# seung-lab/crackle

Hardware: AMD Instinct MI355X
Metric: voxels/s encode+decode, 1024x1024x512 uint32; bit-exact .ckl bytes (higher is better)
Workload: dtype u32

## Files before the change

crackle_amd/_lib.py:

```python
import ctypes as C
import os

HERE = os.path.dirname(os.path.abspath(__file__))
LIB_PATH = os.path.join(HERE, "libcrackle_amd_tuning.so" if os.environ.get("CKL_TUNING_LIB") else
                        ("libcrackle_amd_%s.so" % os.environ["CKL_LIB_AB"]) if os.environ.get("CKL_LIB_AB") else "libcrackle_amd.so")

CKL_OK, CKL_ERR_FORMAT, CKL_ERR_RUNTIME, CKL_ERR_ARG, CKL_ERR_NO_DEVICE, CKL_ERR_CRC = range(6)
MEM_HOST, MEM_DEVICE = 0, 1
CKL_DUST_BINARY_IMAGE, CKL_DUST_INVERT = 1, 2
CKL_ERODE_KEEP_BORDER = 1


class HeaderInfo(C.Structure):
  _fields_ = [
    ("format_version", C.c_uint32), ("label_format", C.c_uint32), ("crack_format", C.c_uint32),
    ("is_signed", C.c_uint32), ("data_width", C.c_uint32), ("stored_data_width", C.c_uint32),
    ("sx", C.c_uint32), ("sy", C.c_uint32), ("sz", C.c_uint32),
    ("fortran_order", C.c_uint32), ("markov_model_order", C.c_uint32), ("is_sorted", C.c_uint32),
    ("num_label_bytes", C.c_uint64), ("header_bytes", C.c_uint64),
  ]


MERGE_UNIQUE_FN = C.CFUNCTYPE(C.c_int, C.c_void_p, C.POINTER(C.c_uint64), C.c_uint64, C.POINTER(C.c_void_p), C.POINTER(C.c_uint64))


class EncodeOverrides(C.Structure):
  _fields_ = [
    ("force_crack_format", C.c_int32), ("force_label_format", C.c_int32),
    ("force_stored_width", C.c_int32), ("has_model", C.c_int32),
    ("model", C.c_void_p),
    ("merge_unique", MERGE_UNIQUE_FN), ("merge_ctx", C.c_void_p),
  ]


EXPORTS = {
  "ckl_last_error": (C.c_char_p, []),
  "ckl_abi_version": (C.c_int, []),
  "ckl_device_count": (C.c_int, []),
  "ckl_header_info_from_bytes": (C.c_int, [C.c_char_p, C.c_uint64, C.POINTER(HeaderInfo)]),
  "ckl_compress": (C.c_int, [
    C.c_void_p, C.c_int, C.c_int, C.c_int, C.c_int64, C.c_int64, C.c_int64,
    C.c_int, C.c_int, C.c_uint64, C.c_int, C.c_int, C.c_int64,
    C.c_int, C.POINTER(C.c_void_p), C.POINTER(C.c_uint64)]),
  "ckl_free": (None, [C.c_void_p]),
  "ckl_decompress": (C.c_int, [
    C.c_void_p, C.c_uint64, C.c_void_p, C.c_uint64, C.c_int,
    C.c_int64, C.c_int64, C.c_int, C.c_uint64, C.c_int]),
  "ckl_decoder_create": (C.c_int, [C.c_void_p, C.c_uint64, C.c_int64, C.c_int64, C.c_int, C.POINTER(C.c_void_p)]),
  "ckl_decoder_create_device": (C.c_int, [C.c_void_p, C.c_uint64, C.c_int64, C.c_int64, C.c_int, C.POINTER(C.c_void_p)]),
  "ckl_encoder_keep_device_stream": (C.c_int, [C.c_void_p, C.c_int]),
  "ckl_encoder_async_host_copy": (C.c_int, [C.c_void_p, C.c_int]),
  "ckl_encoder_host_wait": (C.c_int, [C.c_void_p]),
  "ckl_encoder_device_stream": (C.c_int, [C.c_void_p, C.POINTER(C.c_void_p), C.POINTER(C.c_uint64)]),
  "ckl_decoder_run": (C.c_int, [C.c_void_p, C.c_void_p, C.c_uint64, C.c_int, C.c_uint64]),
  "ckl_decoder_cutout": (C.c_int, [C.c_void_p, C.c_int64, C.c_int64, C.c_int64, C.c_int64, C.c_void_p, C.c_uint64, C.c_int, C.c_uint64]),
  "ckl_cutout": (C.c_int, [
    C.c_void_p, C.c_uint64, C.c_void_p, C.c_uint64, C.c_int,
    C.c_int64, C.c_int64, C.c_int64, C.c_int64, C.c_int64, C.c_int64, C.c_int, C.c_uint64, C.c_int]),
  "ckl_paste": (C.c_int, [
    C.c_void_p, C.c_uint64, C.c_void_p, C.c_int, C.c_int, C.c_uint64,
    C.c_int64, C.c_int64, C.c_int64, C.c_int64, C.c_int64, C.c_int64,
    C.c_int, C.POINTER(C.c_void_p), C.POINTER(C.c_uint64)]),
  "ckl_decoder_label_stats": (C.c_int, [C.c_void_p, C.c_uint64, C.c_void_p, C.c_void_p, C.c_void_p, C.c_void_p, C.POINTER(C.c_uint64)]),
  "ckl_decoder_contacts": (C.c_int, [C.c_void_p, C.POINTER(C.c_void_p), C.POINTER(C.c_void_p), C.POINTER(C.c_uint64)]),
  "ckl_decoder_overlaps": (C.c_int, [C.c_void_p, C.c_void_p, C.POINTER(C.c_void_p), C.POINTER(C.c_void_p), C.POINTER(C.c_uint64)]),
  "ckl_overlaps": (C.c_int, [
    C.c_void_p, C.c_uint64, C.c_void_p, C.c_uint64, C.c_int64, C.c_int64, C.c_int,
    C.POINTER(C.c_void_p), C.POINTER(C.c_void_p), C.POINTER(C.c_uint64)]),
  "ckl_decoder_last_timing": (C.c_int, [C.c_void_p, C.POINTER(C.c_float), C.POINTER(C.c_float)]),
  "ckl_decoder_stage_timing": (C.c_int, [C.c_void_p, C.c_int, C.POINTER(C.c_char_p), C.POINTER(C.c_float)]),
  "ckl_decoder_set_stage_events": (C.c_int, [C.c_void_p, C.c_int]),
  "ckl_decoder_destroy": (None, [C.c_void_p]),
  "ckl_encoder_create": (C.c_int, [C.c_int64, C.c_int64, C.c_int64, C.c_int, C.c_int, C.POINTER(C.c_void_p)]),
  "ckl_encoder_run": (C.c_int, [
    C.c_void_p, C.c_void_p, C.c_int64, C.c_int64, C.c_int64,
    C.c_int, C.c_int, C.c_uint64, C.c_int, C.c_int, C.c_int64,
    C.POINTER(EncodeOverrides), C.POINTER(C.c_void_p), C.POINTER(C.c_uint64)]),
  "ckl_encoder_stats": (C.c_int, [
    C.c_void_p, C.c_void_p, C.c_int64, C.c_int64, C.c_int64,
    C.POINTER(C.c_uint64), C.POINTER(C.c_uint64), C.POINTER(C.c_uint64), C.POINTER(C.c_uint64)]),
  "ckl_encoder_markov_stats": (C.c_int, [
    C.c_void_p, C.c_void_p, C.c_int64, C.c_int64, C.c_int64, C.c_int, C.c_uint64, C.c_void_p]),
  "ckl_encoder_components": (C.c_int, [
    C.c_void_p, C.c_void_p, C.c_int64, C.c_int64, C.c_int64, C.c_uint32, C.c_void_p, C.c_void_p]),
  "ckl_encoder_components_device": (C.c_int, [
    C.c_void_p, C.c_void_p, C.c_int64, C.c_int64, C.c_int64, C.c_uint32, C.c_void_p, C.c_void_p]),
  "ckl_encoder_pin_labels": (C.c_int, [
    C.c_void_p, C.c_void_p, C.c_void_p, C.c_int64, C.c_int64, C.c_int64, C.c_void_p,
    C.c_int, C.c_int, C.c_int64, C.POINTER(C.c_void_p), C.POINTER(C.c_uint64)]),
  "ckl_pins_rows_first": (C.c_int, [C.c_void_p, C.c_void_p, C.c_void_p, C.c_int64, C.c_int64, C.c_int64, C.c_int64, C.c_uint64, C.c_void_p, C.c_void_p, C.c_void_p]),
  "ckl_pins_rows_best": (C.c_int, [C.c_void_p, C.c_void_p, C.c_void_p, C.c_int64, C.c_int64, C.c_int64, C.c_int64, C.c_uint64, C.c_void_p, C.c_void_p]),
  "ckl_pins_rows_extent": (C.c_int, [C.c_void_p, C.c_void_p, C.c_void_p, C.c_int64, C.c_int64, C.c_int64, C.c_int64, C.c_uint64, C.c_void_p, C.c_void_p, C.c_void_p, C.c_void_p]),
  "ckl_pins_rows_ids": (C.c_int, [C.c_void_p, C.c_void_p, C.c_int64, C.c_int64, C.c_int64, C.c_int64, C.c_uint64, C.c_void_p, C.c_void_p, C.c_void_p, C.c_void_p]),
  "ckl_pins_rows_section": (C.c_int, [C.c_void_p, C.c_int64, C.c_int64, C.c_int64, C.c_uint64, C.c_void_p, C.c_void_p, C.c_void_p, C.c_void_p, C.c_void_p, C.c_void_p, C.c_void_p,
                                       C.c_int, C.c_int, C.c_int64, C.POINTER(C.c_void_p), C.POINTER(C.c_uint64)]),
  "ckl_encoder_walk_step_kinds": (C.c_int, [C.c_void_p, C.POINTER(C.c_uint32), C.c_uint32, C.POINTER(C.c_uint32)]),
  "ckl_encoder_last_timing": (C.c_int, [C.c_void_p, C.POINTER(C.c_float), C.POINTER(C.c_float)]),
  "ckl_encoder_walk_paths": (C.c_int, [C.c_void_p, C.POINTER(C.c_uint32), C.POINTER(C.c_uint32)]),
  "ckl_encoder_emit_path": (C.c_int, [C.c_void_p, C.POINTER(C.c_int), C.POINTER(C.c_uint64)]),
  "ckl_encoder_destroy": (None, [C.c_void_p]),
  "ckl_pin_labels_host": (C.c_int, [
    C.c_void_p, C.c_int, C.c_void_p, C.c_int64, C.c_int64, C.c_int64, C.c_void_p,
    C.c_int, C.c_int, C.c_int64, C.POINTER(C.c_void_p), C.POINTER(C.c_uint64)]),
  "ckl_zstack": (C.c_int, [C.POINTER(C.c_char_p), C.POINTER(C.c_uint64), C.c_uint64, C.POINTER(C.c_void_p), C.POINTER(C.c_uint64)]),
  "ckl_decoder_check": (C.c_int, [C.c_void_p, C.c_void_p, C.c_uint64]),
  "ckl_decoder_vcg": (C.c_int, [C.c_void_p, C.c_void_p, C.c_uint64, C.c_int]),
  "ckl_voxel_connectivity_graph": (C.c_int, [C.c_void_p, C.c_uint64, C.c_int, C.c_int, C.c_void_p, C.c_uint64]),
  "ckl_voxel_connectivity_graph_range": (C.c_int, [C.c_void_p, C.c_uint64, C.c_int64, C.c_int64, C.c_int, C.c_int, C.c_void_p, C.c_uint64]),
  "ckl_point_cloud": (C.c_int, [
    C.c_void_p, C.c_uint64, C.c_int64, C.c_int64, C.c_void_p, C.c_uint64, C.c_int, C.c_int, C.c_int,
    C.POINTER(C.c_void_p), C.POINTER(C.c_void_p), C.POINTER(C.c_void_p), C.POINTER(C.c_uint64)]),
  "ckl_reencode_markov": (C.c_int, [C.c_void_p, C.c_uint64, C.c_int, C.c_int, C.POINTER(C.c_void_p), C.POINTER(C.c_uint64)]),
  "ckl_recompress": (C.c_int, [C.c_void_p, C.c_uint64, C.c_int, C.c_int, C.POINTER(C.c_void_p), C.POINTER(C.c_uint64)]),
  "ckl_erode": (C.c_int, [C.c_void_p, C.c_uint64, C.c_int, C.c_int, C.c_int, C.c_int, C.POINTER(C.c_void_p), C.POINTER(C.c_uint64)]),
  "ckl_dilate": (C.c_int, [C.c_void_p, C.c_uint64, C.c_int, C.c_int, C.c_int, C.c_int, C.POINTER(C.c_void_p), C.POINTER(C.c_uint64)]),
  "ckl_decoder_crack_planes": (C.c_int, [C.c_void_p, C.POINTER(C.c_void_p), C.POINTER(C.c_void_p), C.POINTER(C.c_uint32), C.POINTER(C.c_uint64)]),
  "ckl_zsplit": (C.c_int, [C.c_void_p, C.c_uint64, C.c_int64, C.c_int64, C.POINTER(C.c_void_p), C.POINTER(C.c_uint64)]),
  "ckl_encoder_defer_codes": (C.c_int, [C.c_void_p, C.c_int]),
  "ckl_encoder_codes_to_host": (C.c_int, [C.c_void_p, C.c_void_p, C.c_uint64, C.POINTER(C.c_uint64)]),
  "ckl_host_register": (C.c_int, [C.c_void_p, C.c_uint64]),
  "ckl_host_unregister": (C.c_int, [C.c_void_p]),
  "ckl_array_equal": (C.c_int, [C.c_void_p, C.c_uint64, C.c_void_p, C.c_uint64, C.c_int, C.POINTER(C.c_int)]),
  "ckl_mode_pooling_2x2x1": (C.c_int, [C.c_void_p, C.c_uint64, C.c_int64, C.c_int64, C.c_int, C.POINTER(C.c_void_p), C.POINTER(C.c_uint64), C.POINTER(C.c_void_p), C.POINTER(C.c_uint64)]),
  "ckl_connected_components": (C.c_int, [C.c_void_p, C.c_uint64, C.c_int, C.c_int, C.POINTER(C.c_void_p), C.POINTER(C.c_uint64), C.POINTER(C.c_void_p), C.POINTER(C.c_uint64)]),
  "ckl_relabel_components": (C.c_int, [C.c_void_p, C.c_uint64, C.c_void_p, C.c_uint64, C.POINTER(C.c_void_p), C.POINTER(C.c_uint64)]),
  "ckl_dust": (C.c_int, [C.c_void_p, C.c_uint64, C.c_uint64, C.c_int, C.c_int, C.c_int, C.POINTER(C.c_void_p), C.POINTER(C.c_uint64), C.POINTER(C.c_uint64)]),
  "ckl_fill_holes": (C.c_int, [C.c_void_p, C.c_uint64, C.c_int, C.c_int, C.POINTER(C.c_void_p), C.POINTER(C.c_uint64), C.POINTER(C.c_uint64)]),
  "ckl_relabel_values": (C.c_int, [C.c_void_p, C.c_uint64, C.c_void_p, C.c_uint64, C.POINTER(C.c_void_p), C.POINTER(C.c_uint64)]),
  "ckl_crc32c": (C.c_uint32, [C.c_void_p, C.c_uint64]),
  "ckl_crc32c_combine": (C.c_uint32, [C.c_uint32, C.c_uint32, C.c_uint64]),
}

_lib = None


def lib():
  global _lib
  if _lib is None:
    if not os.path.exists(LIB_PATH):
      raise ImportError(
        f"{LIB_PATH} is missing: build the HIP extension first "
        "(python -m crackle_amd.build, or __graft_entry__.build()). "
        "crackle_amd has no CPU fallback."
      )
    L = C.CDLL(LIB_PATH)
    for name, (res, args) in EXPORTS.items():
      f = getattr(L, name)
      f.restype = res
      f.argtypes = args
    _lib = L
  return _lib


def last_error() -> str:
  return lib().ckl_last_error().decode("utf-8", "replace")


class HostStream:

  def __init__(self, ptr: int, n: int):
    self.ptr, self.n = int(ptr), int(n)

  def __len__(self):
    return self.n

  def view(self) -> memoryview:
    return memoryview((C.c_ubyte * self.n).from_address(self.ptr)).cast("B")

  def tobytes(self) -> bytes:
    return C.string_at(self.ptr, self.n)

  __bytes__ = tobytes

  def __eq__(self, other):
    if isinstance(other, HostStream):
      return self.tobytes() == other.tobytes()
    if isinstance(other, (bytes, bytearray, memoryview)):
      return self.tobytes() == bytes(other)
    return NotImplemented

  def __del__(self):
    try:
# ... 12 lines not shown
```

crackle_amd/csrc/ckl_encode.hip:

```cpp
#include "ckl_encoder.hpp"
#include "ckl_decoder.hpp"
#include "ckl_runs.hpp"
#include "ckl_strips.hpp"
#include "ckl_trail.hpp"
#include "ckl_code_words.hpp"
#include "ckl_recompress.hpp"

#include <algorithm>
#include <atomic>
#include <chrono>
#include <functional>
#include <memory>
#include <mutex>

namespace ckl {

using namespace dev;

template <typename LABEL>
__global__ void __launch_bounds__(kBlock) k_stats(const LABEL* __restrict__ labels, uint64_t voxels, unsigned long long* __restrict__ out ) {
	__shared__ unsigned long long s_max[kWaves], s_pairs[kWaves];
	unsigned long long mx = 0, pairs = 0;
	const uint64_t stride = static_cast<uint64_t>(gridDim.x) * kBlock;
	for (uint64_t i = static_cast<uint64_t>(blockIdx.x) * kBlock + threadIdx.x; i < voxels; i += stride) {
// ... 32 lines not shown
	const uint32_t unit0 = (blockIdx.x * kWaves + wave) * kPlaneUnroll;
	const LABEL* slice = labels + static_cast<uint64_t>(zi) * sy * sx;
	LABEL v[kPlaneUnroll], up[kPlaneUnroll], lf[kPlaneUnroll];
	uint32_t xs[kPlaneUnroll], ys[kPlaneUnroll];
#pragma unroll
	for (uint32_t k = 0; k < kPlaneUnroll; k++) {
		const uint32_t unit = unit0 + k;
		const uint32_t y = unit / chunks_per_row;
		const uint32_t x = (unit - y * chunks_per_row) * 64u + lane;
		xs[k] = x; ys[k] = y;
		const bool valid = unit < units && x < sx;
		const LABEL* row = slice + static_cast<uint64_t>(y) * sx;
		v[k] = valid ? row[x] : LABEL(0);
		up[k] = (valid && y > 0) ? row[static_cast<int64_t>(x) - static_cast<int64_t>(sx)] : v[k];
		lf[k] = (valid && lane == 0 && x > 0) ? row[x - 1] : v[k];
	}
	uint32_t nv = 0, nh = 0;
#pragma unroll
	for (uint32_t k = 0; k < kPlaneUnroll; k++) {
		const uint32_t unit = unit0 + k;
		const bool valid = unit < units && xs[k] < sx;
		LABEL left = __shfl_up(v[k], 1, kWave);
		if (lane == 0) left = lf[k];
		const bool dv = valid && xs[k] > 0 && v[k] != left;
		const bool dh = valid && v[k] != up[k];
		const unsigned long long mv = __ballot(dv), mh = __ballot(dh);
		if (lane == 0 && unit < units) {
			const uint32_t c = xs[k] >> 6;
			const uint64_t wbase = zi * plane_words + static_cast<uint64_t>(ys[k]) * row_words + c * 2u;
			planeV[wbase] = static_cast<uint32_t>(mv);
			planeH[wbase] = static_cast<uint32_t>(mh);
			if (c * 2u + 1u < row_words) {
				planeV[wbase + 1] = static_cast<uint32_t>(mv >> 32);
				planeH[wbase + 1] = static_cast<uint32_t>(mh >> 32);
			}
			nv += __popcll(mv);
			nh += __popcll(mh);
		}
	}
	if (lane == 0) { s_red[wave] = nv; s_red[kWaves + wave] = nh; }
	__syncthreads();
	if (threadIdx.x == 0) {
		uint32_t tv = 0, th = 0;
		for (int w = 0; w < kWaves; w++) { tv += s_red[w]; th += s_red[kWaves + w]; }
		if (tv) atomicAdd(count_v + zi, tv);
		if (th) atomicAdd(count_h + zi, th);
	}
}

constexpr uint32_t kBandRows = 32;

template <typename V, typename T>
__device__ __forceinline__ V nt_load_vec(const T* p) {
	typedef uint32_t u32x4_t __attribute__((ext_vector_type(4)));
	static_assert(sizeof(V) == 16, "one 16-byte vector");
	const u32x4_t raw = __builtin_nontemporal_load(reinterpret_cast<const u32x4_t*>(p));
	V v;
	__builtin_memcpy(&v, &raw, 16);
	return v;
}

template <typename T>
__device__ __forceinline__ T wave_shift_up1_label(T v) {
	if constexpr (sizeof(T) == 8) {
		const uint32_t lo = dev::wave_shift_up1(static_cast<uint32_t>(v), 0u), hi = dev::wave_shift_up1(static_cast<uint32_t>(static_cast<uint64_t>(v) >> 32), 0u);
		return static_cast<T>((static_cast<uint64_t>(hi) << 32) | lo);
	}
	else return static_cast<T>(dev::wave_shift_up1(static_cast<uint32_t>(v), 0u));
}
template <uint32_t G>
__device__ __forceinline__ uint32_t or_over_lane_group(uint32_t v) {
	static_assert(G == 2 || G == 4 || G == 8 || G == 16, "lane groups inside a row of 16");
	if constexpr (G >= 2) v |= dev::dpp_u32<0xB1, 0xF>(0u, v);
	if constexpr (G >= 4) v |= dev::dpp_u32<0x4E, 0xF>(0u, v);
	if constexpr (G >= 8) v |= dev::dpp_u32<0x141, 0xF>(0u, v);
	if constexpr (G >= 16) v |= dev::dpp_u32<0x140, 0xF>(0u, v);
	return v;
}

template <typename LABEL>
__global__ void __launch_bounds__(kBlock) k_label_planes_stream(
	const LABEL* __restrict__ labels, uint32_t sx, uint32_t sy, uint32_t strips, uint32_t bands,
	uint32_t* __restrict__ planeV, uint32_t* __restrict__ planeH, uint32_t row_words, uint64_t plane_words,
	uint32_t* __restrict__ partial, unsigned long long* __restrict__ partial_max, unsigned long long* __restrict__ total_pairs
) {
	if (blockIdx.x == 0 && blockIdx.y == 0 && threadIdx.x == 0) *total_pairs = 0;
	constexpr uint32_t P = 16 / sizeof(LABEL);
	constexpr uint32_t G = 32 / P;
	constexpr uint32_t WPR = 64 / G;
	struct alignas(16) Vec { LABEL v[P]; };
	__shared__ uint32_t s_red[3 * kWaves];
	__shared__ unsigned long long s_max[kWaves];
	__shared__ __attribute__((aligned(16))) uint32_t s_words[kWaves][2][kBandRows * WPR];
	const uint32_t zi = blockIdx.y;
	const uint32_t lane = threadIdx.x & 63u, wave = threadIdx.x >> 6;
	const uint32_t task = blockIdx.x * kWaves + wave;
	uint32_t nv = 0, nh = 0, pairs = 0;
	LABEL mxl = 0;
	if (task < strips * bands) {
		const uint32_t band = __builtin_amdgcn_readfirstlane(task / strips), strip = __builtin_amdgcn_readfirstlane(task - (task / strips) * strips);
		const uint32_t x0 = strip * (64u * P);
		const uint32_t x = x0 + lane * P;
		const uint32_t y0 = band * kBandRows, y1 = min(y0 + kBandRows, sy);
		const bool active = x < sx;
		const uint64_t slice_off = static_cast<uint64_t>(zi) * sy * sx;
		const LABEL* col = labels + slice_off + (active ? x : 0u);
		Vec prev;
#pragma unroll
		for (uint32_t i = 0; i < P; i++) prev.v[i] = 0;
		if (y0 > 0) prev = nt_load_vec<Vec>(col + static_cast<uint64_t>(y0 - 1) * sx);
		uint32_t* sv = s_words[wave][0];
		uint32_t* sh = s_words[wave][1];
		auto edge_of = [&](uint32_t y, bool& have) -> LABEL {
			const uint64_t lin = slice_off + static_cast<uint64_t>(y) * sx + x0;
			have = lin > 0;
			const uint64_t at = have ? lin - 1 : 0;
			if constexpr (sizeof(LABEL) >= 4) return labels[at];
			else {
				const uint64_t byte = at * sizeof(LABEL);
				const uint32_t w = reinterpret_cast<const uint32_t*>(reinterpret_cast<uintptr_t>(labels) & ~static_cast<uintptr_t>(3))[(byte + (reinterpret_cast<uintptr_t>(labels) & 3u)) >> 2];
				return static_cast<LABEL>(w >> (8u * static_cast<uint32_t>((byte + (reinterpret_cast<uintptr_t>(labels) & 3u)) & 3u)));
			}
		};
		constexpr uint32_t kRowsAhead = 4;
		Vec rows[kRowsAhead];
		LABEL edges[kRowsAhead];
		bool have_edges[kRowsAhead];
		auto request = [&](uint32_t r, uint32_t y) {
			const uint32_t yl = y < y1 ? y : y1 - 1u;
			rows[r] = nt_load_vec<Vec>(col + static_cast<uint64_t>(yl) * sx);
			edges[r] = edge_of(yl, have_edges[r]);
		};
#pragma unroll
		for (uint32_t r = 0; r < kRowsAhead; r++) request(r, y0 + r);
#pragma unroll
		for (uint32_t it = 0; it < kBandRows / kRowsAhead; it++) {
			const uint32_t yb = y0 + it * kRowsAhead;
#pragma unroll
			for (uint32_t r = 0; r < kRowsAhead; r++) {
				const uint32_t y = yb + r;
				const Vec cur = rows[r];
				const LABEL edge = edges[r];
				const bool have_edge = have_edges[r];
				request(r, y + kRowsAhead);
				if (y >= y1) continue;
				LABEL left = wave_shift_up1_label(cur.v[P - 1]);
				bool have_left = true;
				if (lane == 0) { left = edge; have_left = have_edge; }
				uint32_t bv = 0, bh = 0;
				if (active) {
#pragma unroll
					for (uint32_t i = 0; i < P; i++) {
						const LABEL l = i ? cur.v[i - 1] : left;
						bv |= (cur.v[i] != l ? 1u : 0u) << i;
						bh |= (cur.v[i] != prev.v[i] ? 1u : 0u) << i;
						mxl = cur.v[i] > mxl ? cur.v[i] : mxl;
					}
					pairs += P - __popc(bv) - ((have_left || (bv & 1u)) ? 0u : 1u);
					if (x == 0) bv &= ~1u;
					if (y == 0) bh = 0u;
				}
				nv += __popc(bv); nh += __popc(bh);
				bv <<= (lane % G) * P; bh <<= (lane % G) * P;
				bv = or_over_lane_group<G>(bv); bh = or_over_lane_group<G>(bh);
				if ((lane % G) == 0) { sv[(y - y0) * WPR + lane / G] = bv; sh[(y - y0) * WPR + lane / G] = bh; }
				prev = cur;
			}
		}
		const uint32_t word0 = x0 >> 5;
		uint32_t* pv = planeV + zi * plane_words;
		uint32_t* ph = planeH + zi * plane_words;
		constexpr uint32_t kVecWords = WPR >= 4 ? 4u : WPR;
		constexpr uint32_t kLanesPerRow = WPR / kVecWords;
		for (uint32_t r0 = 0; r0 < y1 - y0; r0 += 64u / kLanesPerRow) {
			const uint32_t r = r0 + lane / kLanesPerRow, w = (lane % kLanesPerRow) * kVecWords;
			if (r >= y1 - y0) continue;
			const uint64_t at = static_cast<uint64_t>(y0 + r) * row_words + word0 + w;
			if (word0 + w + kVecWords <= row_words && ((at & (kVecWords - 1u)) == 0u) && kVecWords == 4u) {
				*reinterpret_cast<uint4*>(pv + at) = *reinterpret_cast<const uint4*>(sv + r * WPR + w);
				*reinterpret_cast<uint4*>(ph + at) = *reinterpret_cast<const uint4*>(sh + r * WPR + w);
			}
			else {
				for (uint32_t q = 0; q < kVecWords; q++) if (word0 + w + q < row_words) { pv[at + q] = sv[r * WPR + w + q]; ph[at + q] = sh[r * WPR + w + q]; }
			}
		}
	}
	nv = wave_sum(nv); nh = wave_sum(nh); pairs = wave_sum(pairs);
	unsigned long long mx = static_cast<unsigned long long>(mxl);
	for (int d = kWave / 2; d >= 1; d >>= 1) { const unsigned long long o = __shfl_xor(mx, d, kWave); mx = o > mx ? o : mx; }
	if (lane == 0) { s_red[wave] = nv; s_red[kWaves + wave] = nh; s_red[2 * kWaves + wave] = pairs; s_max[wave] = mx; }
	__syncthreads();
	if (threadIdx.x == 0) {
		uint32_t tv = 0, th = 0, tp = 0;
		unsigned long long tm = 0;
		for (int w = 0; w < kWaves; w++) { tv += s_red[w]; th += s_red[kWaves + w]; tp += s_red[2 * kWaves + w]; tm = s_max[w] > tm ? s_max[w] : tm; }
		const uint64_t o = static_cast<uint64_t>(zi) * gridDim.x + blockIdx.x;
		partial[o * 4 + 0] = tv; partial[o * 4 + 1] = th; partial[o * 4 + 2] = tp; partial[o * 4 + 3] = 0;
		partial_max[o] = tm;
	}
}

__global__ void __launch_bounds__(kBlock) k_planes_from_cracks(
	const uint32_t* __restrict__ crackV, const uint32_t* __restrict__ crackH, uint32_t sx, uint32_t sy,
	uint32_t row_words, uint64_t plane_words, uint32_t permissible,
	uint32_t* __restrict__ planeV, uint32_t* __restrict__ planeH, uint32_t* __restrict__ counts, uint32_t nslices
) {
	__shared__ uint32_t s_red[kWaves];
	const uint32_t zi = blockIdx.y;
	const uint64_t i = static_cast<uint64_t>(blockIdx.x) * kBlock + threadIdx.x;
	uint32_t nv = 0, nh = 0;
	if (i < plane_words) {
		const uint32_t y = static_cast<uint32_t>(i / row_words);
		const uint32_t w = static_cast<uint32_t>(i - static_cast<uint64_t>(y) * row_words);
		const uint32_t left = sx - w * 32u;
		const uint32_t in_row = left >= 32u ? 0xFFFFFFFFu : ((1u << left) - 1u);
		const uint32_t mv = in_row & (w == 0 ? 0xFFFFFFFEu : 0xFFFFFFFFu);
		const uint32_t mh = y >= 1 ? in_row : 0u;
		const uint64_t at = zi * plane_words + i;
		const uint32_t inv = permissible ? 0xFFFFFFFFu : 0u;
		const uint32_t v = (crackV[at] ^ inv) & mv, h = (crackH[at] ^ inv) & mh;
		planeV[at] = v; planeH[at] = h;
		nv = __popc(v); nh = __popc(h);
	}
	nv = block_sum(nv, s_red); nh = block_sum(nh, s_red);
	if (threadIdx.x == 0) {
		if (nv) atomicAdd(counts + zi, nv);
		if (nh) atomicAdd(counts + nslices + zi, nh);
	}
}

__global__ void __launch_bounds__(kBlock) k_planes_reduce(
	const uint32_t* __restrict__ partial, const unsigned long long* __restrict__ partial_max, uint32_t nblk,
	unsigned long long* __restrict__ out ,
	unsigned long long* __restrict__ total_pairs
) {
	__shared__ uint32_t s_red[kWaves];
	__shared__ unsigned long long s_max[kWaves];
	const uint32_t zi = blockIdx.x;
	uint32_t tv = 0, th = 0, tp = 0;
	unsigned long long tm = 0;
	for (uint32_t b = threadIdx.x; b < nblk; b += kBlock) {
		const uint64_t o = static_cast<uint64_t>(zi) * nblk + b;
		tv += partial[o * 4 + 0]; th += partial[o * 4 + 1]; tp += partial[o * 4 + 2];
		const unsigned long long m = partial_max[o];
		tm = m > tm ? m : tm;
	}
	tv = block_sum(tv, s_red); th = block_sum(th, s_red); tp = block_sum(tp, s_red);
	for (int d = kWave / 2; d >= 1; d >>= 1) { const unsigned long long o = __shfl_xor(tm, d, kWave); tm = o > tm ? o : tm; }
	if ((threadIdx.x & 63) == 0) s_max[threadIdx.x >> 6] = tm;
	__syncthreads();
	if (threadIdx.x == 0) {
		for (int w = 0; w < kWaves; w++) tm = s_max[w] > tm ? s_max[w] : tm;
		out[4ull * zi + 0] = tv; out[4ull * zi + 1] = th; out[4ull * zi + 2] = tp; out[4ull * zi + 3] = tm;
		atomicAdd(total_pairs, static_cast<unsigned long long>(tp));
	}
}

enum : uint8_t { CODE_UP = 0, CODE_RIGHT = 1, CODE_DOWN = 2, CODE_LEFT = 3, CODE_NONE = 0xFE, CODE_TOMB = 0xFF };

struct FinishArgs {
	int sx, sy, xw, yw;
	uint32_t z0;
	uint32_t markov;
	const uint64_t* cbase;
	const uint64_t* kbase;
	const uint32_t* n_chains;
	const uint32_t* n_raw;
	const uint32_t* n_valid;
	const uint8_t* cp;
	const uint32_t* chain_node;
	const uint32_t* chain_off;
	const uint32_t* chain_clen;
	uint32_t* chain_order;
	uint32_t* chain_dst;
	uint32_t* chain_vstart;
	uint8_t* fcode;
	uint8_t* dcode;
	const uint64_t* pbase;
	uint8_t* payload;
	const uint64_t* bbase;
	uint8_t* boc;
	uint32_t* payload_len;
	uint32_t* boc_len;
};

__device__ __forceinline__ void put_le_dev(uint8_t* p, uint32_t v, int w) {
	for (int i = 0; i < w; i++) p[i] = static_cast<uint8_t>((v >> (8 * i)) & 0xFF);
}

constexpr int kFinishBlock = 1024;
constexpr int kFinishWaves = kFinishBlock / kWave;

constexpr uint32_t kFinishChains = 2048;

__global__ void __launch_bounds__(kFinishBlock) k_finish(FinishArgs a) {
	__shared__ uint32_t s_scan[kFinishWaves];
	__shared__ uint32_t s_node[kFinishChains], s_clen[kFinishChains], s_off[kFinishChains], s_ord[kFinishChains], s_dst[kFinishChains], s_vst[kFinishChains];
	const uint32_t zi = blockIdx.x + a.z0;
	const int tid = threadIdx.x;
	const uint32_t nch = a.n_chains[zi], nraw = a.n_raw[zi], nvalid = a.n_valid[zi];
	const uint8_t* cp = a.cp + a.cbase[zi];
	uint8_t* fcode = a.fcode + a.cbase[zi];
	const bool staged = nch <= kFinishChains;
	const uint32_t* ch_node = a.chain_node + a.kbase[zi];
	const uint32_t* ch_off = a.chain_off + a.kbase[zi];
	const uint32_t* ch_clen = a.chain_clen + a.kbase[zi];
	uint32_t* order = a.chain_order + a.kbase[zi];
	uint32_t* dst = a.chain_dst + a.kbase[zi];
	uint32_t* vstart = a.chain_vstart + a.kbase[zi];
	if (staged) {
		for (uint32_t c = tid; c < nch; c += kFinishBlock) { s_node[c] = ch_node[c]; s_clen[c] = ch_clen[c]; s_off[c] = ch_off[c]; }
		__syncthreads();
		ch_node = s_node; ch_off = s_off; ch_clen = s_clen; order = s_ord; dst = s_dst; vstart = s_vst;
	}
	const uint32_t sxe = a.sx + 1;

	if (tid == 0) {
		uint32_t v = 0;
		for (uint32_t c = 0; c < nch; c++) { vstart[c] = v; v += ch_clen[c]; }
		for (uint32_t c = 0; c < nch; c++) {
			const uint32_t key = ch_node[c];
			uint32_t p = c;
			while (p > 0 && ch_node[order[p - 1]] > key) { order[p] = order[p - 1]; p--; }
			order[p] = c;
		}
		uint32_t d = 0;
		for (uint32_t i = 0; i < nch; i++) { dst[order[i]] = d; d += ch_clen[order[i]]; }

		uint8_t* b = a.boc + a.bbase[zi];
		uint32_t num_y = 0, index_size = a.yw;
		for (uint32_t i = 0; i < nch;) {
			const uint32_t y = ch_node[order[i]] / sxe;
			uint32_t j = i;
			while (j < nch && ch_node[order[j]] / sxe == y) j++;
			index_size += a.yw + (j - i + 1) * a.xw;
			num_y++;
// ... 743 lines not shown
) {
	__shared__ unsigned long long s_part[kBlock];
	__shared__ uint32_t s_err;
	if (threadIdx.x == 0) s_err = 0;
	const uint32_t per = (nslices + kBlock - 1) / kBlock;
	const uint32_t z0 = threadIdx.x * per, z1 = min(z0 + per, nslices);
	unsigned long long sum = 0;
	uint32_t err = 0;
	for (uint32_t z = z0; z < z1; z++) { sum += static_cast<unsigned long long>(boc_len[z]) + payload_len[z]; err |= slice_err[z]; }
	s_part[threadIdx.x] = sum;
	__syncthreads();
	if (err) atomicOr(&s_err, err);
	if (threadIdx.x == 0) {
		unsigned long long run = 0;
		for (uint32_t i = 0; i < kBlock; i++) { const unsigned long long v = s_part[i]; s_part[i] = run; run += v; }
		report[nslices] = static_cast<uint32_t>(run); report[nslices + 1] = static_cast<uint32_t>(run >> 32);
	}
	__syncthreads();
	unsigned long long off = s_part[threadIdx.x];
	for (uint32_t z = z0; z < z1; z++) {
		const uint32_t len = boc_len[z] + payload_len[z];
		out_off[z] = off;
		report[z] = len;
		off += len;
	}
	if (threadIdx.x == 0) report[nslices + 2] = s_err;
}

__global__ void __launch_bounds__(kBlock) k_gather_codes(
	const uint8_t* __restrict__ boc, const uint64_t* __restrict__ bbase, const uint32_t* __restrict__ boc_len,
	const uint8_t* __restrict__ payload, const uint64_t* __restrict__ pbase, const uint32_t* __restrict__ payload_len,
	const uint64_t* __restrict__ out_off, uint8_t* __restrict__ out
) {
	const uint32_t zi = blockIdx.x;
	uint8_t* o = out + out_off[zi];
	const uint32_t nb = boc_len[zi], np = payload_len[zi];
	const uint8_t* b = boc + bbase[zi];
	const uint8_t* p = payload + pbase[zi];
	for (uint32_t i = threadIdx.x; i < nb; i += kBlock) o[i] = b[i];
	for (uint32_t i = threadIdx.x; i < np; i += kBlock) o[nb + i] = p[i];
}

struct CrcShifts { uint32_t x[8]; };
__global__ void __launch_bounds__(kBlock) k_crc32c_pieces(const uint8_t* __restrict__ data, uint64_t n, uint64_t pad, uint32_t P, CrcShifts sh, uint32_t* __restrict__ parts) {
	__shared__ uint32_t s_tab[256];
	__shared__ uint32_t s_st[kBlock];
	{
		uint32_t c = threadIdx.x;
		for (int k = 0; k < 8; k++) c = (c & 1u) ? (c >> 1) ^ dev::kCrcPoly : (c >> 1);
		s_tab[threadIdx.x] = c;
	}
	__syncthreads();
	const uint64_t f0 = (static_cast<uint64_t>(blockIdx.x) * kBlock + threadIdx.x) * P;
	uint32_t c = 0;
	for (uint32_t g = 0; g < P; g += 16) {
		const int64_t m0 = static_cast<int64_t>(f0 + g) - static_cast<int64_t>(pad);
		uint32_t w[4] = { 0, 0, 0, 0 };
		if (m0 >= 0 && static_cast<uint64_t>(m0) + 16u <= n) __builtin_memcpy(w, data + m0, 16);
		else if (m0 + 16 > 0) for (int b = 0; b < 16; b++) { const int64_t i = m0 + b; if (i >= 0 && static_cast<uint64_t>(i) < n) w[b >> 2] |= static_cast<uint32_t>(data[i]) << (8 * (b & 3)); }
#pragma unroll
		for (int b = 0; b < 16; b++) c = s_tab[(c ^ (w[b >> 2] >> (8 * (b & 3)))) & 0xFFu] ^ (c >> 8);
	}
	s_st[threadIdx.x] = c;
	__syncthreads();
	for (int k = 0; k < 8; k++) {
		const uint32_t stride = 1u << k;
		if ((threadIdx.x & (2u * stride - 1u)) == 0u) s_st[threadIdx.x] = gf_mul(s_st[threadIdx.x], sh.x[k]) ^ s_st[threadIdx.x + stride];
		__syncthreads();
	}
	if (threadIdx.x == 0) parts[blockIdx.x] = s_st[0];
}
__global__ void __launch_bounds__(kBlock) k_crc32c_fold(const uint32_t* __restrict__ parts, uint32_t G, CrcShifts sh, uint32_t init_term, uint32_t* __restrict__ out) {
	__shared__ uint32_t s_st[kBlock];
	s_st[threadIdx.x] = threadIdx.x < G ? parts[threadIdx.x] : 0u;
	__syncthreads();
	for (int k = 0; (1u << k) < G; k++) {
		const uint32_t stride = 1u << k;
		if ((threadIdx.x & (2u * stride - 1u)) == 0u && threadIdx.x + stride < G) s_st[threadIdx.x] = gf_mul(s_st[threadIdx.x], sh.x[k]) ^ s_st[threadIdx.x + stride];
		__syncthreads();
	}
	if (threadIdx.x == 0) out[0] = ~(s_st[0] ^ init_term);
}

__global__ void __launch_bounds__(kBlock) k_copy_bytes(const uint8_t* __restrict__ src, uint8_t* __restrict__ dst, uint64_t n) {
	const uint64_t head = min(n, static_cast<uint64_t>((4u - (reinterpret_cast<uintptr_t>(dst) & 3u)) & 3u));
	const uint64_t words = (n - head) / 4u;
	const uint64_t tid = static_cast<uint64_t>(blockIdx.x) * kBlock + threadIdx.x;
	const uint64_t stride = static_cast<uint64_t>(gridDim.x) * kBlock;
	if (tid < head) dst[tid] = src[tid];
	const uint64_t tail0 = head + words * 4u;
	if (tid < n - tail0) dst[tail0 + tid] = src[tail0 + tid];
	const uint8_t* s0 = src + head;
	const uint32_t sh = static_cast<uint32_t>(reinterpret_cast<uintptr_t>(s0) & 3u) * 8u;
	const uint32_t* sw = reinterpret_cast<const uint32_t*>(reinterpret_cast<uintptr_t>(s0) & ~static_cast<uintptr_t>(3));
	uint32_t* dw = reinterpret_cast<uint32_t*>(dst + head);
	if (sh == 0u) {
		for (uint64_t i = tid; i < words; i += stride) dw[i] = sw[i];
	}
	else {
		for (uint64_t i = tid; i < words; i += stride) dw[i] = __funnelshift_r(sw[i], sw[i + 1], sh);
	}
}

__global__ void __launch_bounds__(kBlock) k_trail_step_kinds(const uint32_t* __restrict__ events, const uint64_t* __restrict__ ibase, const uint32_t* __restrict__ n_events, uint32_t* __restrict__ counts) {
	__shared__ uint32_t s_c[5];
	const uint32_t zi = blockIdx.x;
	if (threadIdx.x < 5) s_c[threadIdx.x] = 0u;
	__syncthreads();
	const uint32_t n = n_events[zi] & ~(dev::kEvFormatAddr12 | dev::kEvWalkWide);
	const uint32_t* ev = events + ibase[zi];
	uint32_t c[4] = { 0, 0, 0, 0 };
	for (uint32_t i = threadIdx.x; i < n; i += kBlock) c[ev[i] >> 30]++;
	for (int k = 0; k < 4; k++) if (c[k]) atomicAdd(&s_c[k], c[k]);
	if (threadIdx.x == 0) {
		uint32_t run = 0, longest = 0;
		for (uint32_t i = 0; i < n; i++) { if ((ev[i] >> 30) == 1u) run = 0; else { run++; longest = run > longest ? run : longest; } }
		s_c[4] = longest;
	}
	__syncthreads();
	if (threadIdx.x < 5) counts[zi * 5u + threadIdx.x] = s_c[threadIdx.x];
}

}

using namespace ckl;

static void crc32c_device(const uint8_t* data, uint64_t n, uint32_t* parts, uint32_t* out, hipStream_t s) {
	uint32_t P = 128, G = 1;
	while (G < static_cast<uint32_t>(kBlock) && static_cast<uint64_t>(G) * kBlock * P < n) G <<= 1;
	if (static_cast<uint64_t>(G) * kBlock * P < n) P = static_cast<uint32_t>(((n + static_cast<uint64_t>(G) * kBlock - 1) / (static_cast<uint64_t>(G) * kBlock) + 15) / 16 * 16);
	const uint64_t frame = static_cast<uint64_t>(G) * kBlock * P;
	static std::mutex shifts_mutex;
	static uint32_t shifts_for = 0;
	static CrcShifts shifts_in, shifts_over;
	CrcShifts in_wg, over_wg;
	{
		std::lock_guard<std::mutex> lock(shifts_mutex);
		if (shifts_for != P) {
			for (int k = 0; k < 8; k++) {
				shifts_in.x[k] = gf_xpow(8ull * P << k);
				shifts_over.x[k] = gf_xpow(8ull * P * kBlock << k);
			}
			shifts_for = P;
		}
		in_wg = shifts_in; over_wg = shifts_over;
	}
	hipLaunchKernelGGL(k_crc32c_pieces, dim3(G), dim3(kBlock), 0, s, data, n, frame - n, P, in_wg, parts);
	hipLaunchKernelGGL(k_crc32c_fold, dim3(1), dim3(kBlock), 0, s, parts, G, over_wg, gf_mul(0xFFFFFFFFu, gf_xpow(8ull * n)), out);
}

static void copy_bytes_device(const uint8_t* src, uint8_t* dst, uint64_t n, hipStream_t s) {
	if (!n) return;
	const uint32_t blocks = static_cast<uint32_t>(std::min<uint64_t>((n / 4u + kBlock - 1) / kBlock + 1u, 8192u));
	hipLaunchKernelGGL(k_copy_bytes, dim3(blocks), dim3(kBlock), 0, s, src, dst, n);
}

namespace {

struct UploadPacker {
	struct Item { void* buf; size_t off, count; void (*bind)(void*, uint8_t*, size_t); };
	std::vector<Item> items;
	std::vector<uint8_t> image;
	template <typename T>
	void add(DevBuf<T>& dst, const std::vector<T>& src) {
		const size_t off = (image.size() + 255) & ~static_cast<size_t>(255);
		image.resize(off + std::max<size_t>(src.size(), 1) * sizeof(T));
		if (!src.empty()) memcpy(image.data() + off, src.data(), src.size() * sizeof(T));
		items.push_back({ &dst, off, src.size(), [](void* b, uint8_t* base, size_t n) { static_cast<DevBuf<T>*>(b)->borrow(reinterpret_cast<T*>(base), n); } });
	}
	void commit(DevBuf<uint8_t>& block, hipStream_t s, void** staging = nullptr) {
		if (image.empty()) return;
		for (const Item& it : items) it.bind(it.buf, nullptr, 0);
		block.ensure(image.size());
		if (staging) {
			if (*staging) host_out_free(*staging);
			*staging = host_out_alloc(std::max<size_t>(image.size(), 64u << 10));
			memcpy(*staging, image.data(), image.size());
			upload_small(block.p, *staging, image.size(), s, *staging);
		}
		else CKL_HIP(hipMemcpyAsync(block.p, image.data(), image.size(), hipMemcpyHostToDevice, s));
		for (const Item& it : items) it.bind(it.buf, block.p + it.off, it.count);
	}
};

template <typename LABEL>
VolumeStats volume_stats(ckl_encoder& e, const LABEL* labels, uint64_t voxels) {
	VolumeStats st;
	if (voxels == 0) return st;
	hipStream_t s = e.stream;
	e.d_stats.ensure(2);
	CKL_HIP(hipMemsetAsync(e.d_stats.p, 0, 2 * sizeof(unsigned long long), s));
	const uint32_t blocks = static_cast<uint32_t>(std::min<uint64_t>((voxels + kBlock - 1) / kBlock, 256ull * 8));
	hipLaunchKernelGGL(k_stats<LABEL>, dim3(blocks), dim3(kBlock), 0, s, labels, voxels, e.d_stats.p);
	auto r = download(e.d_stats.p, 2, s);
	st.max_label = r[0]; st.pairs = r[1];
	LABEL f, l;
	CKL_HIP(hipMemcpy(&f, labels, sizeof(LABEL), hipMemcpyDeviceToHost));
	CKL_HIP(hipMemcpy(&l, labels + (voxels - 1), sizeof(LABEL), hipMemcpyDeviceToHost));
	st.first = f; st.last = l;
	return st;
}

inline bool planes_cached(const ckl_encoder& e, const void* labels, int64_t sx, int64_t sy, int64_t sz) {
	return e.planes_for == labels && e.planes_dims[0] == sx && e.planes_dims[1] == sy && e.planes_dims[2] == sz;
}

inline uint64_t crack_edges(const ckl_encoder& e, int64_t sx, int64_t sy, size_t zi, bool permissible) {
	const uint64_t interior = static_cast<uint64_t>(sx > 0 ? sx - 1 : 0) * sy + static_cast<uint64_t>(sx) * (sy > 0 ? sy - 1 : 0);
	const uint64_t differ = static_cast<uint64_t>(e.count_v[zi]) + e.count_h[zi];
	return permissible ? interior - differ : differ;
}

void planes_collect(ckl_encoder& e, uint32_t ns, VolumeStats* st, const std::vector<unsigned long long>* fetched = nullptr) {
	std::vector<unsigned long long> mine;
	if (!fetched) { mine = download(e.d_plane_out.p, 4ull * ns, e.stream); fetched = &mine; }
	const std::vector<unsigned long long>& o = *fetched;
	e.count_v.resize(ns); e.count_h.resize(ns);
	VolumeStats v;
	for (uint32_t zi = 0; zi < ns; zi++) {
		e.count_v[zi] = static_cast<uint32_t>(o[4ull * zi]);
		e.count_h[zi] = static_cast<uint32_t>(o[4ull * zi + 1]);
		v.pairs += o[4ull * zi + 2];
		v.max_label = std::max<uint64_t>(v.max_label, o[4ull * zi + 3]);
	}
	e.planes_deferred = false;
	if (st) *st = v;
}

void trail_prezero(ckl_encoder& e, int64_t sx, int64_t sy, int64_t sz) {
	hipStream_t s = e.stream2;
	const uint32_t ns = static_cast<uint32_t>(sz);
	const uint64_t nverts = static_cast<uint64_t>(sx + 1) * (sy + 1);
	const uint32_t start_words = static_cast<uint32_t>((nverts + 31) / 32);
	e.d_slice_err.ensure(ns);
	e.t_counters.ensure(7 * static_cast<size_t>(ns));
	e.t_start_bits.ensure(static_cast<size_t>(start_words) * ns);
	CKL_HIP(hipMemsetAsync(e.d_slice_err.p, 0, ns * sizeof(uint32_t), s));
	CKL_HIP(hipMemsetAsync(e.t_counters.p, 0, 7 * static_cast<size_t>(ns) * sizeof(uint32_t), s));
	CKL_HIP(hipMemsetAsync(e.t_start_bits.p, 0, static_cast<size_t>(start_words) * ns * sizeof(uint32_t), s));
	CKL_HIP(hipEventRecord(e.ev_prezero, s));
	e.trail_zeroed = true;
}

template <typename LABEL>
void planes_pass(ckl_encoder& e, const LABEL* labels, int64_t sx, int64_t sy, int64_t sz, VolumeStats* st, bool defer = false) {
	hipStream_t s = e.stream;
	const uint32_t ns = static_cast<uint32_t>(sz);
	e.trail_zeroed = false;
	e.planes_deferred = false;
	e.row_words = static_cast<uint32_t>((sx + 31) / 32);
	e.plane_words = static_cast<uint64_t>(e.row_words) * sy;
	e.d_planes.ensure(2 * e.plane_words * ns);
	constexpr uint32_t P = 16 / sizeof(LABEL);
	const bool fast = !getenv("CKL_PLANES_GENERIC") && sx >= static_cast<int64_t>(P) && sx % P == 0 && (reinterpret_cast<uintptr_t>(labels) & 15u) == 0;
	if (fast) {
		const uint32_t strips = static_cast<uint32_t>((sx + 64 * P - 1) / (64 * P));
		const uint32_t bands = static_cast<uint32_t>((sy + kBandRows - 1) / kBandRows);
		const uint32_t nblk = (strips * bands + kWaves - 1) / kWaves;
		e.d_plane_partial.ensure(4ull * nblk * ns);
		e.d_plane_partial_max.ensure(static_cast<size_t>(nblk) * ns);
		e.d_plane_out.ensure(4ull * ns + 1);
		trail_prezero(e, sx, sy, sz);
		hipLaunchKernelGGL(k_label_planes_stream<LABEL>, dim3(nblk, ns), dim3(kBlock), 0, s,
			labels, static_cast<uint32_t>(sx), static_cast<uint32_t>(sy), strips, bands,
			plane_v(e), plane_h(e, ns), e.row_words, e.plane_words,
			e.d_plane_partial.p, e.d_plane_partial_max.p, e.d_plane_out.p + 4ull * ns);
		hipLaunchKernelGGL(k_planes_reduce, dim3(ns), dim3(kBlock), 0, s, e.d_plane_partial.p, e.d_plane_partial_max.p, nblk, e.d_plane_out.p, e.d_plane_out.p + 4ull * ns);
		e.planes_deferred = defer;
		if (!e.planes_deferred) planes_collect(e, ns, st);
		return;
	}
	if (st) *st = volume_stats<LABEL>(e, labels, static_cast<uint64_t>(sx) * sy * sz);
	e.d_count_vh.ensure(2 * static_cast<size_t>(ns));
	CKL_HIP(hipMemsetAsync(e.d_count_vh.p, 0, 2 * static_cast<size_t>(ns) * sizeof(uint32_t), s));
	const uint32_t chunks = static_cast<uint32_t>((sx + 63) / 64);
	const uint64_t units = static_cast<uint64_t>(chunks) * sy;
	hipLaunchKernelGGL(k_label_planes<LABEL>, dim3(static_cast<uint32_t>((units + kWaves * kPlaneUnroll - 1) / (kWaves * kPlaneUnroll)), ns), dim3(kBlock), 0, s,
		labels, static_cast<uint32_t>(sx), static_cast<uint32_t>(sy), chunks,
		plane_v(e), plane_h(e, ns), e.row_words, e.plane_words,
		e.d_count_vh.p, e.d_count_vh.p + ns);
	std::vector<uint32_t> c = download(e.d_count_vh.p, 2 * static_cast<size_t>(ns), s);
	e.count_v.assign(c.begin(), c.begin() + ns);
	e.count_h.assign(c.begin() + ns, c.end());
}

void planes_pass_any(ckl_encoder& e, const void* labels, int64_t sx, int64_t sy, int64_t sz, VolumeStats* st) {
	with_label_type(e.dtype_bytes, [&](auto t) { planes_pass(e, static_cast<const typename decltype(t)::type*>(labels), sx, sy, sz, st); });
}

enum class GraphFormat : uint32_t { IMPERMISSIBLE = 0, PERMISSIBLE = 1, ON_DEVICE = 2 };
inline GraphFormat graph_format(bool permissible) { return permissible ? GraphFormat::PERMISSIBLE : GraphFormat::IMPERMISSIBLE; }
void graph_pass(ckl_encoder& e, int64_t sx, int64_t sy, int64_t sz, GraphFormat format, VolumeStats* st = nullptr) {
	hipStream_t s = e.stream;
	const uint32_t ns = static_cast<uint32_t>(sz);
	e.tiles_x = static_cast<uint32_t>((sx + 1 + kTrailTileDim - 1) / kTrailTileDim);
	e.tiles_y = static_cast<uint32_t>((sy + 1 + 7) / 8);
	const uint32_t mtx = static_cast<uint32_t>((sx + 1 + 7) / 8), mty = static_cast<uint32_t>((sy + 1 + 7) / 8);
	e.mtx2 = (mtx + 1) / 2;
	e.adjm_stride = static_cast<uint64_t>(e.mtx2) * ((mty + 1) / 2) * 4 * 2;
	e.d_adjm.ensure(e.adjm_stride * ns);
	e.graph_blocks = (e.tiles_x * e.tiles_y + kBlock - 1) / kBlock;
	e.t_blk_special.ensure(static_cast<size_t>(e.graph_blocks) * ns);
	e.t_blk_corner.ensure(static_cast<size_t>(e.graph_blocks) * ns);
	e.d_count_vh.ensure(4 * static_cast<size_t>(ns));
	const bool on_device = format == GraphFormat::ON_DEVICE;
	if (on_device && !e.planes_deferred) throw Error(CKL_ERR_RUNTIME, "crackle_amd: internal: crack format left to the device without deferred counts");
	const unsigned long long half_voxels = static_cast<unsigned long long>(static_cast<int64_t>(static_cast<uint64_t>(sx) * sy * sz) / 2);
	hipLaunchKernelGGL(k_trail_graph, dim3(e.graph_blocks, ns), dim3(kBlock), 0, s,
		plane_v(e), plane_h(e, ns), e.row_words, e.plane_words,
		static_cast<uint32_t>(sx), static_cast<uint32_t>(sy), static_cast<uint32_t>(format),
		on_device ? e.d_plane_out.p + 4ull * ns : nullptr, half_voxels,
		reinterpret_cast<uint32_t*>(e.d_adjm.p), e.adjm_stride * 4,
		e.mtx2, e.tiles_x, e.tiles_y, e.t_blk_special.p, e.t_blk_corner.p);
	hipLaunchKernelGGL(k_trail_count_scan, dim3(ns), dim3(kBlock), 0, s, e.t_blk_special.p, e.t_blk_corner.p, e.graph_blocks,
		e.d_count_vh.p + 2 * static_cast<size_t>(ns), e.d_count_vh.p + 3 * static_cast<size_t>(ns));
	std::vector<unsigned long long> po;
	if (e.planes_deferred) {
		po.resize(4ull * ns);
		CKL_HIP(hipMemcpyAsync(po.data(), e.d_plane_out.p, po.size() * sizeof(unsigned long long), hipMemcpyDeviceToHost, s));
	}
	std::vector<uint32_t> c = download(e.d_count_vh.p + 2 * static_cast<size_t>(ns), 2 * static_cast<size_t>(ns), s);
	e.count_special.assign(c.begin(), c.begin() + ns);
	e.count_corner.assign(c.begin() + ns, c.end());
	VolumeStats v;
	if (!po.empty()) planes_collect(e, ns, &v, &po);
	if (st && !po.empty()) *st = v;
	e.graph_permissible = on_device ? static_cast<int64_t>(v.pairs) < static_cast<int64_t>(static_cast<uint64_t>(sx) * sy * sz) / 2 : format == GraphFormat::PERMISSIBLE;
}

enum class CrackGoal { HISTOGRAM, CODES };
struct CrackRequest {
	CrackGoal goal = CrackGoal::CODES;
	bool permissible = false;
	int markov_order = 0;
	const std::vector<uint8_t>* model = nullptr;
	bool reuse_trail = false;
	std::function<void()> overlap;
};
struct CrackResult {
	std::vector<uint32_t> code_len;
	uint64_t total = 0;
	bool any_chain = false;
	std::vector<uint32_t> hist;
	std::vector<uint8_t> model;
};

inline size_t trail_walk_lds(uint32_t max_special) { return (static_cast<size_t>(max_special) + 256) * 16 + 1024; }

constexpr size_t kEmitLdsCap = 80 * 1024;
struct EmitPlan {
	bool fused = false;
	uint32_t tcap = 0, wcap = 0;
	size_t dyn = 0, need = 0;
};
EmitPlan emit_plan(uint64_t max_edges, uint32_t max_kcap, int max_lds) {
	EmitPlan p;
	static const size_t static_lds = [] {
		hipFuncAttributes fattr;
		CKL_HIP(hipFuncGetAttributes(&fattr, reinterpret_cast<const void*>(&k_trail_emit)));
		return static_cast<size_t>(fattr.sharedSizeBytes);
	}();
	p.tcap = std::min<uint32_t>(kFinishChains, ((max_kcap + 15u) / 16u) * 16u);
	const uint64_t words = (max_edges + max_edges / 8 + 1024 + 15) / 16;
	p.wcap = static_cast<uint32_t>(std::min<uint64_t>(words, 1u << 28));
	if (const char* env = getenv("CKL_TRAIL_EMIT_WORDS")) p.wcap = static_cast<uint32_t>(std::max(1, std::min<int>(atoi(env), static_cast<int>(p.wcap))));
	p.dyn = 4 * (2 * static_cast<size_t>(p.tcap) + std::max<size_t>(3 * static_cast<size_t>(p.tcap), p.wcap));
	p.need = static_lds + p.dyn;
	size_t cap = kEmitLdsCap;
	if (const char* env = getenv("CKL_TRAIL_EMIT_LDS")) cap = static_cast<size_t>(std::max(0, atoi(env)));
	cap = std::min(cap, static_cast<size_t>(std::max(0, max_lds)));
	const char* sw = getenv("CKL_TRAIL_EMIT");
	p.fused = !(sw && !strcmp(sw, "0")) && words < (1u << 28) && p.need <= cap;
	return p;
}

FinishArgs finish_args(const ckl_encoder& e, int64_t sx, int64_t sy, int markov_order) {
	FinishArgs fa;
	fa.sx = static_cast<int>(sx); fa.sy = static_cast<int>(sy);
	fa.xw = byte_width(static_cast<uint64_t>(sx) + 1); fa.yw = byte_width(static_cast<uint64_t>(sy) + 1);
	fa.markov = markov_order ? 1u : 0u;
	fa.cbase = e.d_cbase.p; fa.kbase = e.d_kbase.p;
	fa.n_chains = e.d_n_chains.p; fa.n_raw = e.d_n_raw.p; fa.n_valid = e.d_n_valid.p;
	fa.cp = e.d_cp.p; fa.chain_node = e.d_chain_node.p; fa.chain_off = e.d_chain_off.p; fa.chain_clen = e.d_chain_clen.p;
	fa.chain_order = e.d_chain_order.p; fa.chain_dst = e.d_chain_dst.p; fa.chain_vstart = e.d_chain_vstart.p;
	fa.fcode = e.d_fcode.p; fa.dcode = e.d_dcode.p;
	fa.pbase = e.d_pbase.p; fa.payload = e.d_payload.p; fa.bbase = e.d_bbase.p; fa.boc = e.d_boc.p;
	fa.payload_len = e.d_payload_len.p; fa.boc_len = e.d_boc_len.p;
	fa.z0 = 0;
	return fa;
}

TrailArgs trail_args(const ckl_encoder& e, int64_t sx, int64_t sy, uint32_t ns) {
	const uint64_t nverts = static_cast<uint64_t>(sx + 1) * (sy + 1);
	TrailArgs ta;
	ta.adjm = e.d_adjm.p; ta.adjm_stride = e.adjm_stride; ta.mtx2 = e.mtx2; ta.tiles_x = e.tiles_x; ta.tiles_y = e.tiles_y;
	ta.planeV = plane_v(e); ta.planeH = plane_h(e, ns); ta.row_words = e.row_words; ta.plane_words = e.plane_words;
	ta.sx = static_cast<uint32_t>(sx); ta.sy = static_cast<uint32_t>(sy); ta.inv = e.graph_permissible ? 0xFFFFFFFFu : 0u;
	ta.sxe = static_cast<uint32_t>(sx + 1); ta.sye = static_cast<uint32_t>(sy + 1); ta.nverts = static_cast<uint32_t>(nverts);
	ta.max_steps = e.t_max_steps.p;
	ta.nbase = e.t_nbase.p; ta.ncap = e.t_ncap.p;
	ta.n_nodes = e.t_counters.p; ta.n_corners = e.t_counters.p + 2 * ns;
	ta.n_starts = e.t_counters.p + 3 * ns; ta.n_items = e.t_counters.p + 4 * ns;
	ta.node_vertex = e.t_node_vertex.p; ta.node_adj = e.t_node_adj.p; ta.vert2node = e.t_vert2node.p;
	ta.cobase = e.t_cobase.p; ta.cocap = e.t_cocap.p; ta.corner_vertex = e.t_corner_vertex.p;
	ta.dart_end = e.t_dart_end.p; ta.dart_len = e.t_dart_len.p; ta.dart_minv = e.t_dart_minv.p; ta.dart_minpos = e.t_dart_minpos.p;
	ta.dart_codes = e.t_dart_codes.p; ta.dart_inline = e.t_dart_inline.p;
	ta.parent = e.t_parent.p; ta.compmin = e.t_compmin.p;
	ta.start_bits = e.t_start_bits.p; ta.start_words = static_cast<uint32_t>((nverts + 31) / 32); ta.starts = e.t_starts.p;
	ta.ibase = e.t_ibase.p; ta.icap = e.t_icap.p; ta.items = e.t_items.p; ta.item_off = e.t_item_off.p;
	ta.sbase = e.d_sbase.p; ta.scap = e.d_scap.p; ta.stack_node = e.d_stack_node.p; ta.stack_item = e.d_stack_code.p;
	ta.kbase = e.d_kbase.p; ta.kcap = e.d_kcap.p;
	ta.chain_node = e.d_chain_node.p; ta.chain_item0 = e.t_chain_item0.p; ta.chain_off = e.d_chain_off.p; ta.chain_clen = e.d_chain_clen.p;
	ta.n_chains = e.d_n_chains.p; ta.n_raw = e.d_n_raw.p; ta.n_valid = e.d_n_valid.p;
	ta.cbase = e.d_cbase.p; ta.ccap = e.d_ccap.p; ta.cp = e.d_cp.p; ta.slice_err = e.d_slice_err.p;
	ta.events = e.t_events.p; ta.n_events = e.t_counters.p + 5 * ns; ta.seg_len_sum = e.t_counters.p + 6 * ns; ta.chain_ev0 = e.t_chain_ev0.p; ta.ev_lnd = e.t_ev_lnd.p; ta.ev_item = e.t_ev_item.p;
	ta.dbg = nullptr;
	{ const char* env = getenv("CKL_TRAIL_WALK"); ta.walk_plain = (env && !strcmp(env, "plain")) ? 1u : 0u; ta.walk_no_regs = (env && !strcmp(env, "lds")) ? 1u : 0u; }
	{ const char* env = getenv("CKL_TRAIL_WALK_STACK"); ta.walk_stack_cap = env ? static_cast<uint32_t>(std::max(1, atoi(env))) : 0xFFFFFFFFu; }
	ta.graph_blocks = e.graph_blocks; ta.blk_special = e.t_blk_special.p; ta.blk_corner = e.t_blk_corner.p;
	ta.z0 = 0;
	return ta;
}

void trail_diag(ckl_encoder& e, uint32_t ns, const unsigned long long* ta_dbg, uint32_t max_special, size_t trail_lds_used) {
	hipStream_t s = e.stream;
	std::vector<uint32_t> c = download(e.t_counters.p, 5 * static_cast<size_t>(ns), s);
	double m[5] = { 0 };
	for (int k = 0; k < 5; k++) for (uint32_t zi = 0; zi < ns; zi++) m[k] += static_cast<double>(c[static_cast<size_t>(k) * ns + zi]) / ns;
	double sp = 0, co = 0;
	for (uint32_t zi = 0; zi < ns; zi++) { sp += static_cast<double>(e.count_special[zi]) / ns; co += static_cast<double>(e.count_corner[zi]) / ns; }
	if (ta_dbg) {
		std::vector<unsigned long long> g = download(ta_dbg, 16, s);
		if (g[11]) fprintf(stderr, "[ckl trail diag, k_trail_walk] mean cycles per slice: table fill=%.0f fill + walk=%.0f\n", static_cast<double>(g[6]) / g[11], static_cast<double>(g[7]) / g[11]);
		if (g[11]) fprintf(stderr, "[ckl trail diag, k_trail_walk] slices=%llu iterations/slice=%.0f cycles/iteration=%.0f clock=%.2f GHz (cycles / 100 MHz ticks)\n",
			g[11], static_cast<double>(g[8]) / g[11], g[8] ? static_cast<double>(g[9]) / g[8] : 0.0, g[10] ? static_cast<double>(g[9]) / (g[10] * 10.0) : 0.0);
		fprintf(stderr, "[ckl trail diag, k_trail_components, mean cycles per slice] union=%.0f component minima=%.0f starts/splits=%.0f bitmap scan=%.0f\n",
			static_cast<double>(g[12]) / ns, static_cast<double>(g[13]) / ns, static_cast<double>(g[14]) / ns, static_cast<double>(g[15]) / ns);
		fprintf(stderr, "[ckl trail diag, k_trail_segments] waves=%llu iterations/wave mean=%.1f max=%llu cycles/wave mean=%.0f max=%llu cycles/iteration=%.0f active lanes/iteration=%.1f\n",
			g[4], g[4] ? static_cast<double>(g[0]) / g[4] : 0.0, g[1], g[4] ? static_cast<double>(g[2]) / g[4] : 0.0, g[3],
			g[0] ? static_cast<double>(g[2]) / g[0] : 0.0, g[0] ? static_cast<double>(g[5]) / g[0] : 0.0);
	}
	fprintf(stderr, "[ckl trail diag] max degree-1/3/4 vertices of a slice=%u, k_trail_walk LDS=%zu bytes\n", max_special, trail_lds_used);
	fprintf(stderr, "[ckl trail diag, mean per slice] degree-1/3/4 vertices=%.0f corners=%.0f nodes=%.0f starts=%.0f items=%.0f\n", sp, co, m[0], m[3], m[4]);
}

void check_walk_errors(ckl_encoder& e, uint32_t ns) {
	const std::vector<uint32_t> errs = download(e.d_slice_err.p, ns, e.stream);
	for (uint32_t zi = 0; zi < ns; zi++) if (errs[zi]) throw Error(CKL_ERR_RUNTIME, "crackle_amd: crack walk scratch overflow on z=" + std::to_string(zi));
}

CrackResult crack_pass(ckl_encoder& e, int64_t sx, int64_t sy, int64_t sz, const CrackRequest& rq) {
	hipStream_t s = e.stream;
	const uint32_t ns = static_cast<uint32_t>(sz);
	const uint64_t nverts = static_cast<uint64_t>(sx + 1) * (sy + 1);
	const int markov_order = rq.markov_order;
	const bool reuse_trail = rq.reuse_trail;
	if (rq.goal == CrackGoal::HISTOGRAM && (!markov_order || rq.model)) throw Error(CKL_ERR_RUNTIME, "crackle_amd: internal: a markov histogram needs an order and no model");
	CrackResult result;
	e.d_slice_err.ensure(ns);
	const bool prezeroed = e.trail_zeroed && !reuse_trail;
	e.trail_zeroed = false;
	if (prezeroed) CKL_HIP(hipStreamWaitEvent(s, e.ev_prezero, 0));
	if (!reuse_trail && !prezeroed) CKL_HIP(hipMemsetAsync(e.d_slice_err.p, 0, ns * sizeof(uint32_t), s));

	std::vector<uint64_t> cbase(ns), sbase(ns), kbase(ns);
	std::vector<uint32_t> ccap(ns), scap(ns), kcap(ns), max_steps(ns);
	std::vector<uint64_t> nbase(ns), cobase(ns), ibase(ns);
	std::vector<uint32_t> ncap(ns), cocap(ns), icap(ns);
	uint64_t ctot = 0, stot = 0, ktot = 0, ntot = 0, cotot = 0, itot = 0;
	uint32_t max_ncap = 0, max_cocap = 0, max_icap = 0, max_special = 0, max_kcap = 0;
	uint64_t max_edges = 0;
	bool any = false;
	for (uint32_t zi = 0; zi < ns; zi++) {
		const uint64_t E = crack_edges(e, sx, sy, zi, rq.permissible);
		any = any || E > 0;
		const uint64_t cc = ((7 * E + 16 + 15) / 16) * 16;
		if (cc > 0xFFFFFFF0ull) throw Error(CKL_ERR_RUNTIME, "crackle_amd: slice has too many crack edges");
		cbase[zi] = ctot; ccap[zi] = static_cast<uint32_t>(cc); ctot += cc;
		max_steps[zi] = static_cast<uint32_t>(E + 1);
		const uint64_t nc = ((static_cast<uint64_t>(e.count_special[zi]) + e.count_corner[zi] + 16) / 16) * 16;
		if (nc >= (1ull << 28)) throw Error(CKL_ERR_RUNTIME, "crackle_amd: slice has too many crack vertices");
		nbase[zi] = ntot; ncap[zi] = static_cast<uint32_t>(nc); ntot += nc;
		cobase[zi] = cotot; cocap[zi] = e.count_corner[zi]; cotot += e.count_corner[zi];
		const uint64_t ic = 7 * nc + 16;
		ibase[zi] = itot; icap[zi] = static_cast<uint32_t>(ic); itot += ic;
		sbase[zi] = stot; scap[zi] = static_cast<uint32_t>(2 * nc + 4); stot += 2 * nc + 4;
		kbase[zi] = ktot; kcap[zi] = static_cast<uint32_t>(nc); ktot += nc;
		max_ncap = std::max<uint32_t>(max_ncap, ncap[zi]);
		max_cocap = std::max<uint32_t>(max_cocap, cocap[zi]);
		max_icap = std::max<uint32_t>(max_icap, icap[zi]);
		max_special = std::max<uint32_t>(max_special, e.count_special[zi]);
		max_kcap = std::max<uint32_t>(max_kcap, kcap[zi]);
		max_edges = std::max<uint64_t>(max_edges, E);
	}
	result.any_chain = any;
	if (g_ht && g_ht->on) {
		uint32_t over = 0;
		for (uint32_t zi = 0; zi < ns; zi++) over += e.count_special[zi] > 3584u;
		fprintf(stderr, "[ckl trail nodes] max special %u, slices above 3584: %u of %u\n", max_special, over, ns);
	}
	HT_MARK("c:caps");

	UploadPacker tables;
	tables.add(e.d_cbase, cbase); tables.add(e.d_ccap, ccap);
	tables.add(e.d_sbase, sbase); tables.add(e.d_scap, scap);
	tables.add(e.d_kbase, kbase); tables.add(e.d_kcap, kcap);
	int max_lds = 0;
	CKL_HIP(hipDeviceGetAttribute(&max_lds, hipDeviceAttributeMaxSharedMemoryPerBlock, e.device));
	EmitPlan emit;
	if (!reuse_trail) {
		emit = emit_plan(max_edges, max_kcap, max_lds);
		e.emit_fused = emit.fused; e.emit_lds = emit.need;
		if (!emit.fused) { e.d_cp.ensure(ctot); e.d_fcode.ensure(ctot); e.d_chain_clen.ensure(ktot); e.d_chain_vstart.ensure(ktot); }
	}
	if (markov_order) e.d_dcode.ensure(ctot);
	e.d_stack_node.ensure(stot); e.d_stack_code.ensure(stot);
	e.d_chain_node.ensure(ktot); e.d_chain_off.ensure(ktot);
	e.d_chain_order.ensure(ktot); e.d_chain_dst.ensure(ktot);
	e.d_n_chains.ensure(ns); e.d_n_raw.ensure(ns); e.d_n_valid.ensure(ns);
	e.d_payload_len.ensure(ns); e.d_boc_len.ensure(ns);
	const int xw = byte_width(static_cast<uint64_t>(sx) + 1), yw = byte_width(static_cast<uint64_t>(sy) + 1);
	std::vector<uint64_t> pbase(ns), bbase(ns);
	uint64_t ptot = 0, btot = 0;
	for (uint32_t zi = 0; zi < ns; zi++) {
		const uint64_t ncodes = ccap[zi];
		const uint64_t pbytes = markov_order ? (3ull * ncodes + 2 + 7) / 8 : (ncodes + 3) / 4;
		pbase[zi] = ptot; ptot += ((pbytes + 8 + 3) / 4) * 4;
		const uint64_t bbytes = 4 + yw + static_cast<uint64_t>(kcap[zi]) * (yw + 2 * xw);
		bbase[zi] = btot; btot += bbytes;
	}
	tables.add(e.d_pbase, pbase); tables.add(e.d_bbase, bbase);
	tables.add(e.t_nbase, nbase); tables.add(e.t_ncap, ncap);
	tables.add(e.t_cobase, cobase); tables.add(e.t_cocap, cocap);
	tables.add(e.t_ibase, ibase); tables.add(e.t_icap, icap);
	tables.add(e.t_max_steps, max_steps);
	tables.commit(e.d_crack_tables, s, e.uploads_by_kernel ? &e.tables_staging : nullptr);
	HT_MARK("c:tables");
	e.d_payload.ensure(ptot + 8); e.d_boc.ensure(btot + 8);
	e.codes_capacity = ptot + btot;
	if (markov_order) CKL_HIP(hipMemsetAsync(e.d_payload.p, 0, ptot + 8, s));

	DevBuf<unsigned long long> d_tdbg;
	size_t trail_lds_used = 0;
	if (!reuse_trail) {
		e.t_counters.ensure(7 * static_cast<size_t>(ns));
		if (!prezeroed) CKL_HIP(hipMemsetAsync(e.t_counters.p, 0, 7 * static_cast<size_t>(ns) * sizeof(uint32_t), s));
		e.t_node_vertex.ensure(ntot); e.t_node_adj.ensure(ntot + 16); e.t_vert2node.ensure(nverts * ns);
		e.t_corner_vertex.ensure(cotot);
		e.t_dart_end.ensure(4 * ntot); e.t_dart_len.ensure(4 * ntot); e.t_dart_minv.ensure(4 * ntot); e.t_dart_minpos.ensure(4 * ntot);
		e.t_dart_codes.ensure(4 * ntot); e.t_dart_inline.ensure(4 * ntot);
		e.t_parent.ensure(ntot); e.t_compmin.ensure(ntot); e.t_starts.ensure(ntot);
		const uint32_t start_words = static_cast<uint32_t>((nverts + 31) / 32);
		e.t_start_bits.ensure(static_cast<size_t>(start_words) * ns);
		if (!prezeroed) CKL_HIP(hipMemsetAsync(e.t_start_bits.p, 0, static_cast<size_t>(start_words) * ns * sizeof(uint32_t), s));
		e.t_items.ensure(itot); e.t_item_off.ensure(itot); e.t_chain_item0.ensure(ktot);
		e.t_events.ensure(itot); e.t_chain_ev0.ensure(ktot); e.t_ev_lnd.ensure(itot); e.t_ev_item.ensure(itot);
		e.last_trail_slices = ns;

		TrailArgs ta = trail_args(e, sx, sy, ns);
		const FinishArgs fa = finish_args(e, sx, sy, markov_order);
		if (kTuning && getenv("CKL_TRAIL_DIAG")) { d_tdbg.ensure(16); CKL_HIP(hipMemsetAsync(d_tdbg.p, 0, 128, s)); ta.dbg = d_tdbg.p; }
		const size_t budget = static_cast<size_t>(max_lds > 1024 ? max_lds - 1024 : 0);
		const uint32_t dart_blocks = (4 * max_ncap + kWalkChunk * kWaves - 1) / (kWalkChunk * kWaves);
		size_t clds = (static_cast<size_t>(max_special) + 1024) * 12;
		if (const char* env = getenv("CKL_TRAIL_LDS")) clds = static_cast<size_t>(std::max(0, atoi(env)));
		clds = (std::min(budget, std::max<size_t>(clds, 1024)) / 16) * 16;
		CKL_HIP(hipFuncSetAttribute(reinterpret_cast<const void*>(&k_trail_components), hipFuncAttributeMaxDynamicSharedMemorySize, static_cast<int>(clds)));
		size_t lds = trail_walk_lds(max_special);
		if (const char* env = getenv("CKL_TRAIL_LDS")) lds = static_cast<size_t>(std::max(0, atoi(env)));
		lds = std::min(budget, std::max<size_t>(lds, 4096));
		lds = (lds / 16) * 16;
		CKL_HIP(hipFuncSetAttribute(reinterpret_cast<const void*>(&k_trail_walk), hipFuncAttributeMaxDynamicSharedMemorySize, static_cast<int>(lds)));
		trail_lds_used = lds;
		HT_MARK("c:setup");

		if (any) {
			hipLaunchKernelGGL(k_trail_nodes, dim3(e.graph_blocks, ns), dim3(kBlock), 0, s, ta);
			hipLaunchKernelGGL(k_trail_segments, dim3(dart_blocks, ns), dim3(kBlock), 0, s, ta);
			if (max_cocap) hipLaunchKernelGGL(k_trail_loops, dim3((max_cocap + kBlock - 1) / kBlock, ns), dim3(kBlock), 0, s, ta);
			hipLaunchKernelGGL(k_trail_components, dim3(ns), dim3(kCompBlock), clds, s, ta, static_cast<uint32_t>(clds));
		}
		CKL_HIP(hipEventRecord(e.evd0, s));
		hipLaunchKernelGGL(k_trail_walk, dim3(ns), dim3(kWave), lds, s, ta, static_cast<uint32_t>(lds));
		CKL_HIP(hipEventRecord(e.evd1, s));
		hipLaunchKernelGGL(k_trail_items, dim3(ns), dim3(kItemsBlock), 0, s, ta);
		if (emit.fused) {
			CKL_HIP(hipFuncSetAttribute(reinterpret_cast<const void*>(&k_trail_emit), hipFuncAttributeMaxDynamicSharedMemorySize, static_cast<int>(emit.dyn)));
			hipLaunchKernelGGL(k_trail_emit, dim3(ns), dim3(kEmitBlock), emit.dyn, s, ta, fa, emit.tcap, emit.wcap);
		}
		else {
			hipLaunchKernelGGL(k_trail_offsets, dim3(ns), dim3(kBlock), 0, s, ta);
			hipLaunchKernelGGL(k_trail_expand, dim3((max_icap + kExpandChunk * kWaves - 1) / (kExpandChunk * kWaves), ns), dim3(kBlock), 0, s, ta);
			hipLaunchKernelGGL(k_finish, dim3(ns), dim3(kFinishBlock), 0, s, fa);
		}
	}
	HT_MARK("c:enqueue");
	if (kTuning && getenv("CKL_TRAIL_DIAG")) trail_diag(e, ns, d_tdbg.p, max_special, trail_lds_used);

	auto enqueue_tail = [&]() {
		e.d_out_off.ensure(ns);
		e.d_code_report.ensure(static_cast<size_t>(ns) + 3);
		e.d_codes_out.ensure(e.codes_capacity + 8);
		hipLaunchKernelGGL(k_code_offsets, dim3(1), dim3(kBlock), 0, s, e.d_boc_len.p, e.d_payload_len.p, e.d_slice_err.p, ns, e.d_out_off.p, e.d_code_report.p);
		hipLaunchKernelGGL(k_gather_codes, dim3(ns), dim3(kBlock), 0, s, e.d_boc.p, e.d_bbase.p, e.d_boc_len.p,
			e.d_payload.p, e.d_pbase.p, e.d_payload_len.p, e.d_out_off.p, e.d_codes_out.p);
	};
	if (!markov_order) enqueue_tail();
	if (rq.overlap) rq.overlap();
	HT_MARK("c:overlap");

	if (markov_order) {
		if (rq.model) result.model = *rq.model;
		else {
			const size_t rows = static_cast<size_t>(1) << (2 * markov_order);
			e.d_hist.ensure(rows * 4);
			CKL_HIP(hipMemsetAsync(e.d_hist.p, 0, rows * 4 * sizeof(uint32_t), s));
			const uint32_t hist_lds = (rows * 4 <= 16384) ? static_cast<uint32_t>(rows * 4) : 0u;
			if (hist_lds * 4 > 48 * 1024) CKL_HIP(hipFuncSetAttribute(reinterpret_cast<const void*>(&k_markov_hist), hipFuncAttributeMaxDynamicSharedMemorySize, static_cast<int>(hist_lds * 4)));
			hipLaunchKernelGGL(k_markov_hist, dim3(ns), dim3(kBlock), hist_lds * sizeof(uint32_t), s, e.d_dcode.p, e.d_cbase.p, e.d_n_valid.p, markov_order, e.d_hist.p, hist_lds);
			result.hist = download(e.d_hist.p, rows * 4, s);
			if (rq.goal == CrackGoal::HISTOGRAM) { check_walk_errors(e, ns); return result; }
			result.model = markov_stats_to_model(result.hist.data(), rows);
		}
		upload(e.d_model, result.model, s);
		hipLaunchKernelGGL(k_markov_pack, dim3(ns), dim3(kBlock), 0, s, e.d_dcode.p, e.d_cbase.p, e.d_n_valid.p, markov_order,
			e.d_model.p, e.d_pbase.p, e.d_payload.p, e.d_payload_len.p);
		enqueue_tail();
	}
	HT_MARK("c:finish_enq");
	const std::vector<uint32_t> report = download(e.d_code_report.p, static_cast<size_t>(ns) + 3, s);
	HT_MARK("c:finish_wait");
	if (report[ns + 2]) check_walk_errors(e, ns);
	result.code_len.assign(report.begin(), report.begin() + ns);
	result.total = static_cast<uint64_t>(report[ns]) | (static_cast<uint64_t>(report[ns + 1]) << 32);
	return result;
}

struct FlatResult {
	std::vector<uint32_t> ncomp;
	std::vector<uint32_t> crcs;
	uint64_t total = 0;
};

void ensure_geom_table(ckl_encoder& e, uint64_t sxy) {
	if (e.g_table_pixels == sxy && e.d_G.p) return;
	hipStream_t s = e.stream2;
	const uint32_t npx = static_cast<uint32_t>(sxy);
	const uint32_t B = 1024, nblk = npx / B + 1;
	std::vector<uint32_t> g_base(B), blk_g(nblk), blk_x(nblk);
	const uint32_t X = gf_xpow(32);
	g_base[0] = 0;
	for (uint32_t i = 1; i < B; i++) g_base[i] = gf_mul(X, g_base[i - 1] ^ 0x80000000u);
	const uint32_t gB = gf_mul(X, g_base[B - 1] ^ 0x80000000u);
	const uint32_t XB = gf_xpow(32ull * B);
	blk_g[0] = 0; blk_x[0] = 0x80000000u;
	for (uint32_t k = 1; k < nblk; k++) {
		blk_g[k] = blk_g[k - 1] ^ gf_mul(blk_x[k - 1], gB);
		blk_x[k] = gf_mul(blk_x[k - 1], XB);
	}
	DevBuf<uint32_t> t_base, t_g, t_x;
	upload(t_base, g_base, s); upload(t_g, blk_g, s); upload(t_x, blk_x, s);
	e.d_G.ensure(static_cast<size_t>(npx) + 1);
	hipLaunchKernelGGL(k_build_geom_table, dim3(npx / kBlock + 1), dim3(kBlock), 0, s, t_base.p, t_g.p, t_x.p, npx, e.d_G.p);
	CKL_HIP(hipStreamSynchronize(s));
	e.g_table_pixels = sxy;
}

RunArrays flat_arrays(const ckl_encoder& e) {
	RunArrays ra;
	ra.word_base = e.d_word_base.p; ra.rbase = e.d_rbase.p; ra.rcap = e.d_rcap.p;
	ra.parent = e.d_parent.p; ra.run_start = e.d_run_start.p; ra.run_cc = e.d_run_cc.p;
	ra.nruns = e.d_nruns.p; ra.ncomp = e.d_ncomp.p; ra.slice_err = e.d_slice_err2.p;
	ra.comp_pix = e.d_comp_pix.p;
	return ra;
}

void flat_report_layout(ckl_encoder& e, uint32_t ns, hipStream_t s) {
	e.d_flat_report.ensure(4 * static_cast<size_t>(ns) + 1);
	e.d_ncomp.borrow(e.d_flat_report.p, ns); e.d_crc_acc.borrow(e.d_flat_report.p + ns, ns);
	e.d_idbits.borrow(e.d_flat_report.p + 2 * static_cast<size_t>(ns), ns); e.d_slice_err2.borrow(e.d_flat_report.p + 3 * static_cast<size_t>(ns), ns);
	CKL_HIP(hipMemsetAsync(e.d_slice_err2.p, 0, (static_cast<size_t>(ns) + 1) * sizeof(uint32_t), s));
}

RunGeom flat_geom(const ckl_encoder& e, int64_t sx, int64_t sy, uint32_t ns) {
	RunGeom g;
	g.planeV = plane_v(e); g.planeH = plane_h(e, ns);
	g.row_words = e.row_words; g.plane_words = e.plane_words;
	g.flip = 1u;
	g.sx = static_cast<uint32_t>(sx); g.sy = static_cast<uint32_t>(sy);
	return g;
}

void flat_enqueue_runs(ckl_encoder& e, int64_t sx, int64_t sy, int64_t sz) {
	hipStream_t s = e.stream2;
	const uint32_t ns = static_cast<uint32_t>(sz);
	const uint64_t sxy = static_cast<uint64_t>(sx) * sy;
	e.flat_strips = false;

	std::vector<uint64_t>& rbase = e.h_rbase;
	std::vector<uint32_t>& rcap = e.h_rcap;
	rbase.assign(ns, 0); rcap.assign(ns, 0);
	uint64_t rtot = 0;
	uint32_t max_rcap = 0;
	for (uint32_t zi = 0; zi < ns; zi++) {
		const uint64_t runs = static_cast<uint64_t>(sy) + e.count_v[zi];
		rbase[zi] = rtot; rcap[zi] = static_cast<uint32_t>(runs); rtot += runs;
		max_rcap = std::max<uint32_t>(max_rcap, static_cast<uint32_t>(runs));
	}
	upload(e.d_rbase, rbase, s); upload(e.d_rcap, rcap, s);
	e.d_word_base.ensure(e.plane_words * ns);
	e.d_parent.ensure(rtot); e.d_run_start.ensure(rtot); e.d_run_cc.ensure(rtot); e.d_comp_pix.ensure(rtot);
	e.d_nruns.ensure(ns);
	flat_report_layout(e, ns, s);
// ... 181 lines not shown
		for (; j >= 2048; j >>= 1) hipLaunchKernelGGL(k_bitonic_step, dim3(blocks), dim3(kBlock), 0, s, e.d_sorted.p, j, k, n_pad);
		hipLaunchKernelGGL(k_bitonic_local, dim3(n_pad / 2048), dim3(kBlock), 0, s, e.d_sorted.p, j, k, n_pad);
	}
	{
		const uint32_t ub = static_cast<uint32_t>((n_sort + kUniqItems - 1) / kUniqItems);
		e.d_uniq_blk.ensure(ub + 1);
		hipLaunchKernelGGL(k_unique_count, dim3(ub), dim3(kBlock), 0, s, e.d_sorted.p, static_cast<uint32_t>(n_sort), e.d_uniq_blk.p);
		hipLaunchKernelGGL(k_unique_scan, dim3(1), dim3(kBlock), 0, s, e.d_uniq_blk.p, ub, e.d_n_uniq.p);
		hipLaunchKernelGGL(k_unique_scatter, dim3(ub), dim3(kBlock), 0, s, e.d_sorted.p, static_cast<uint32_t>(n_sort), e.d_uniq_blk.p, e.d_uniq.p);
	}
	}
	uint64_t uniq_bound = N;
	const bool merged_list = ov && ov->merge_unique;
	if (ov && ov->merge_unique) {
		HT_MARK("l:enqueue");
		const uint32_t n_local = merge_unsorted ? static_cast<uint32_t>(n_sort) : download(e.d_n_uniq.p, 1, s)[0];
		std::vector<uint64_t> local = download(merge_unsorted ? e.d_label_list.p : e.d_uniq.p, n_local, s);
		HT_MARK("l:local");
		const uint64_t* merged = nullptr;
		uint64_t n_merged = 0;
		if (ov->merge_unique(ov->merge_ctx, local.data(), n_local, &merged, &n_merged) != 0 || (!merged && n_merged))
			throw Error(CKL_ERR_RUNTIME, "crackle_amd: the merge_unique callback failed");
		HT_MARK("l:merge");
		if (n_merged < n_local || n_merged > 0xFFFFFFFFull) throw Error(CKL_ERR_ARG, "crackle_amd: merge_unique returned a list that cannot contain the slab's labels");
		e.d_uniq.ensure(n_merged + 1);
		if (n_merged) CKL_HIP(hipMemcpyAsync(e.d_uniq.p, merged, n_merged * sizeof(uint64_t), hipMemcpyHostToDevice, s));
		const uint32_t nm[2] = { static_cast<uint32_t>(n_merged), 0u };
		CKL_HIP(hipMemcpyAsync(e.d_n_uniq.p, nm, sizeof(nm), hipMemcpyHostToDevice, s));
		CKL_HIP(hipStreamSynchronize(s));
		e.d_labels_bin.ensure(8 + n_merged * static_cast<uint64_t>(stored_width) + static_cast<uint64_t>(ns) * component_width + N * 4 + 16);
		uniq_bound = std::max<uint64_t>(uniq_bound, n_merged);
	}
	e.d_labels_bin.ensure(8 + N * static_cast<uint64_t>(stored_width) + static_cast<uint64_t>(ns) * component_width + N * 4 + 16);
	const uint64_t work = std::max<uint64_t>(std::max<uint64_t>(uniq_bound, ns), 1);
	hipLaunchKernelGGL(k_flat_section, dim3(static_cast<uint32_t>((work + kBlock - 1) / kBlock)), dim3(kBlock), 0, s,
		e.d_uniq.p, e.d_n_uniq.p, stored_width, e.d_ncomp.p, ns, component_width, e.d_mapping.p, static_cast<uint32_t>(N), e.d_labels_bin.p,
		merged_list ? e.d_n_uniq.p + 1 : nullptr);
	HT_MARK("l:enqueue");
	const std::vector<uint32_t> report = download(e.d_n_uniq.p, merged_list ? 2 : 1, s);
	const uint32_t nu = report[0];
	HT_MARK("l:wait");
	if (merged_list && report[1]) throw Error(CKL_ERR_ARG, "crackle_amd: merge_unique returned a list that lacks a label of the slab");
	return 8 + static_cast<uint64_t>(nu) * stored_width + static_cast<uint64_t>(ns) * component_width + N * static_cast<uint64_t>(byte_width(nu));
}

}

Header ckl::stream_header(int data_width, int64_t sx, int64_t sy, int64_t sz, const VolumeStats& st, bool allow_pins, bool fortran_order, uint64_t markov_model_order, const ckl_encode_overrides* ov) {
	Header head;
	head.crack_format = IMPERMISSIBLE;
	head.label_format = PINS_VARIABLE_WIDTH;
	if (static_cast<int64_t>(st.pairs) < static_cast<int64_t>(static_cast<uint64_t>(sx) * sy * sz) / 2) {
		head.crack_format = PERMISSIBLE;
		head.label_format = FLAT;
	}
	if (ov && ov->force_crack_format >= 0) {
		head.crack_format = ov->force_crack_format;
		head.label_format = ov->force_crack_format == PERMISSIBLE ? FLAT : PINS_VARIABLE_WIDTH;
	}
	if (sz == 1 || !allow_pins) head.label_format = FLAT;
	if (ov && ov->force_label_format >= 0) head.label_format = ov->force_label_format;
	head.is_signed = false;
	head.data_width = data_width;
	head.stored_data_width = ov && ov->force_stored_width ? ov->force_stored_width : byte_width(st.max_label);
	head.sx = static_cast<uint32_t>(sx); head.sy = static_cast<uint32_t>(sy); head.sz = static_cast<uint32_t>(sz);
	head.log2_grid_size = 31;
	head.fortran_order = fortran_order;
	head.markov_model_order = static_cast<int>(markov_model_order & 0xFF);
	head.is_sorted = true;
	return head;
}

void ckl::check_dims(int64_t sx, int64_t sy, int64_t sz, int dtype_bytes, int is_signed) {
	if (is_signed) throw Error(CKL_ERR_ARG, "Signed integer data types are not currently supported.");
	if (dtype_bytes != 1 && dtype_bytes != 2 && dtype_bytes != 4 && dtype_bytes != 8) throw Error(CKL_ERR_ARG, "crackle_amd: dtype width must be 1, 2, 4 or 8 bytes");
	if (sx < 0 || sy < 0 || sz < 0) throw Error(CKL_ERR_ARG, "crackle_amd: negative dimension");
	if (sx > 0x7FFFFFF0ll || sy > 0x7FFFFFF0ll || sz > 0x7FFFFFF0ll) throw Error(CKL_ERR_ARG, "crackle_amd: dimension too large");
	if (static_cast<uint64_t>(sx + 1) * static_cast<uint64_t>(sy + 1) >= (1ull << 30)) throw Error(CKL_ERR_ARG, "crackle_amd: slices of 2^30 or more crack vertices are not supported");
}

void ckl::planes_adopt(ckl_encoder& e, uint32_t row_words, uint64_t plane_words, uint32_t ns, uint32_t count_rows) {
	e.row_words = row_words;
	e.plane_words = plane_words;
	e.d_planes.ensure(2 * plane_words * ns);
	e.d_count_vh.ensure(4 * static_cast<size_t>(ns));
	CKL_HIP(hipMemsetAsync(e.d_count_vh.p, 0, count_rows * static_cast<size_t>(ns) * sizeof(uint32_t), e.stream));
}

void ckl::planes_adopt_counts(ckl_encoder& e, const std::vector<uint32_t>& counts, uint32_t ns) {
	e.count_v.assign(counts.begin(), counts.begin() + ns);
	e.count_h.assign(counts.begin() + ns, counts.begin() + 2 * static_cast<size_t>(ns));
}

namespace {

struct EncodeRequest {
	bool allow_pins = false, fortran_order = false;
	uint64_t markov_model_order = 0;
	bool optimize_pins = false, auto_bgcolor = true;
	int64_t manual_bgcolor = 0;
	const ckl_encode_overrides* overrides = nullptr;
};

template <typename LABEL>
void encode_typed(ckl_encoder& e, const LABEL* labels, int64_t sx, int64_t sy, int64_t sz, const EncodeRequest& req, uint8_t** out, uint64_t* out_len) {
	const ckl_encode_overrides* const ov = req.overrides;
	const uint64_t voxels = static_cast<uint64_t>(sx) * sy * sz;
	hipStream_t s = e.stream;
	CKL_HIP(hipEventRecord(e.ev0, s));

	HostTimer ht;
	g_ht = &ht;
	VolumeStats st;
	e.trail_zeroed = false;
	const bool have_planes = voxels > 0 && (e.label_src ? planes_cached(e, e.label_src, sx, sy, sz) : ov && planes_cached(e, labels, sx, sy, sz));
	e.planes_for = nullptr;
	if (e.label_src && voxels > 0 && !have_planes) throw Error(CKL_ERR_RUNTIME, "crackle_amd: internal: recompress without its planes");
	const bool labels_first = getenv("CKL_NO_OVERLAP") || static_cast<uint64_t>(sx) * sy > (1536ull * 1536ull)
		|| (getenv("CKL_LABELS_AT_WALK") && atoi(getenv("CKL_LABELS_AT_WALK")) == 0);
	if (voxels > 0 && !have_planes) planes_pass<LABEL>(e, labels, sx, sy, sz, &st, !labels_first);
	else if (have_planes) st = e.planes_stats;
	ht.mark("planes");
	bool graph_done = false;
	if (e.planes_deferred) {
		e.trail_for = nullptr;
		graph_pass(e, sx, sy, sz, ov && ov->force_crack_format >= 0 ? graph_format(ov->force_crack_format == PERMISSIBLE) : GraphFormat::ON_DEVICE, &st);
		graph_done = true;
		ht.mark("graph");
	}
	Header head = stream_header(static_cast<int>(sizeof(LABEL)), sx, sy, sz, st, req.allow_pins, req.fortran_order, req.markov_model_order, ov);
	const int stored_width = head.stored_data_width;
	e.uploads_by_kernel = head.label_format == FLAT;
	if (voxels == 0) { hand_out(header_bytes(head), OutAlloc::MALLOC, out, out_len); return; }
	if (req.optimize_pins) throw Error(CKL_ERR_ARG, "crackle_amd: allow_pins=2 (find_optimal_pins) is out of scope");
	if (head.label_format != FLAT && head.label_format != PINS_VARIABLE_WIDTH) throw Error(CKL_ERR_ARG, "crackle_amd: unsupported label format");
	if (head.markov_model_order > 13) throw Error(CKL_ERR_ARG, "crackle_amd: markov_model_order > 13 is not supported on device");

	bool labels_at_walk = false;
	const bool need_runs = head.label_format != FLAT;
	if (labels_first && !graph_done) flat_enqueue(e, labels, sx, sy, sz, need_runs, false);
	const bool trail_cached = !graph_done && have_planes && ov && ov->has_model && head.markov_model_order > 0 && e.trail_for == static_cast<const void*>(labels)
		&& e.trail_perm == (head.crack_format == PERMISSIBLE) && e.trail_order == head.markov_model_order;
	e.trail_for = nullptr;
	if (graph_done && e.graph_permissible != (head.crack_format == PERMISSIBLE)) throw Error(CKL_ERR_RUNTIME, "crackle_amd: internal: device and host disagree on the crack format");
	if (!trail_cached && !graph_done) graph_pass(e, sx, sy, sz, graph_format(head.crack_format == PERMISSIBLE));
	ht.mark("graph");
	if (!labels_first) {
		uint32_t max_special = 0;
		for (uint32_t v : e.count_special) max_special = std::max(max_special, v);
		int max_lds = 0;
		CKL_HIP(hipDeviceGetAttribute(&max_lds, hipDeviceAttributeMaxSharedMemoryPerBlock, e.device));
		labels_at_walk = max_special < 5000 && 2 * trail_walk_lds(max_special) + kFlatResolveLds <= static_cast<size_t>(max_lds);
		if (!labels_at_walk) flat_enqueue(e, labels, sx, sy, sz, need_runs, false);
	}

	const bool permissible = head.crack_format == PERMISSIBLE;
	{
		bool any = false;
		for (int64_t z = 0; z < sz && !any; z++) any = crack_edges(e, sx, sy, z, permissible) > 0;
		if (!any && !(ov && ov->has_model)) head.markov_model_order = 0;
	}
	std::vector<uint8_t> forced_model;
	CrackRequest crq;
	crq.permissible = permissible;
	crq.markov_order = head.markov_model_order;
	crq.reuse_trail = trail_cached;
	if (ov && ov->has_model && head.markov_model_order > 0) {
		const size_t rows = static_cast<size_t>(1) << (2 * head.markov_model_order);
		forced_model.assign(ov->model, ov->model + rows * 4);
		crq.model = &forced_model;
	}

	FlatResult fr;
	std::vector<uint8_t> pins_binary;
	uint64_t label_bytes = 0;
	const uint64_t off_index = Header::kBytes;
	const uint64_t off_labels = off_index + 4ull * (sz + 1);
	uint64_t est_code_bytes = 0;
	{
		const int xw = byte_width(static_cast<uint64_t>(sx) + 1), yw = byte_width(static_cast<uint64_t>(sy) + 1);
		for (int64_t z = 0; z < sz; z++) {
			const uint64_t codes = crack_edges(e, sx, sy, z, permissible) + 4ull * (static_cast<uint64_t>(e.count_special[z]) + e.count_corner[z]) + 16;
			est_code_bytes += (head.markov_model_order ? (3 * codes + 7) / 8 : (codes + 3) / 4) + 8;
			est_code_bytes += 4 + yw + 64ull * (yw + 2 * xw);
		}
	}
	if (getenv("CKL_SMALL_ESTIMATE")) est_code_bytes = 0;
	const uint64_t model_bytes_est = head.markov_model_order ? (1ull << (2 * head.markov_model_order)) : 0;
	struct HostOut { void* p = nullptr; ~HostOut() { if (p) host_out_free(p); } } early;
	uint64_t early_cap = 0;
	uint32_t labels_crc = 0;
	const int component_width = byte_width(static_cast<uint64_t>(sx) * sy);
	hipStream_t s2 = e.stream2;
	bool labels_stay = false;
	auto label_side = [&]() {
		if (labels_at_walk) {
			CKL_HIP(hipStreamWaitEvent(s2, e.evd0, 0));
			flat_enqueue(e, labels, sx, sy, sz, need_runs, true);
		}
		flat_collect<LABEL>(e, labels, sx, sy, sz, fr);
		HT_MARK("flat");
		const uint64_t N = fr.total;
		if (head.label_format == PINS_VARIABLE_WIDTH) {
			if (N > 0xFFFFFFFFull) throw Error(CKL_ERR_RUNTIME, "crackle_amd: too many components");
			e.d_cc_volume.ensure(voxels);
			launch_paint_components(s2, plane_v(e), e.row_words, e.plane_words, sx, sy, sz, e.d_word_base.p, e.d_rbase.p, e.d_run_cc.p, e.d_comp_off.p, 0u, e.d_cc_volume.p);
			pins_binary = pins_section_plain<LABEL>(e, labels, e.d_cc_volume.p, e.d_mapping.p, sx, sy, sz, N, fr.ncomp, head.pin_index_width(), stored_width, req.auto_bgcolor, req.manual_bgcolor);
			label_bytes = pins_binary.size();
		}
		else {
			label_bytes = flat_section(e, N, stored_width, component_width, static_cast<uint32_t>(sz), ov);
			HT_MARK("label_table");
			labels_stay = e.async_host_copy && e.keep_device_stream && !e.defer_codes && label_bytes > 0;
			early_cap = off_labels + label_bytes + model_bytes_est + est_code_bytes + 4ull * (sz + 1) + 64;
			early.p = host_out_alloc(early_cap);
			HT_MARK("l:buffer");
			uint8_t* eo = static_cast<uint8_t*>(early.p);
			if (labels_stay) {
				e.d_labels_crc.ensure(1 + kBlock);
				if (!e.ev_labels_crc) CKL_HIP(hipEventCreateWithFlags(&e.ev_labels_crc, hipEventDisableTiming));
				crc32c_device(e.d_labels_bin.p, label_bytes, e.d_labels_crc.p + 1, e.d_labels_crc.p, s2);
				CKL_HIP(hipEventRecord(e.ev_labels_crc, s2));
			}
			else {
				if (label_bytes) CKL_HIP(hipMemcpyAsync(eo + off_labels, e.d_labels_bin.p, label_bytes, hipMemcpyDeviceToHost, s2));
				CKL_HIP(hipStreamSynchronize(s2));
				labels_crc = crc32c(eo + off_labels, label_bytes);
			}
			HT_MARK("labels_d2h");
		}
	};

	const bool no_overlap = getenv("CKL_NO_OVERLAP") != nullptr;
	if (!no_overlap) crq.overlap = label_side;
	const CrackResult cr = crack_pass(e, sx, sy, sz, crq);
	if (no_overlap) label_side();
	ht.mark("cracks");
	std::vector<uint8_t> stored_model;
	if (head.markov_model_order > 0) stored_model = markov_model_to_stored(cr.model);

	head.num_label_bytes = label_bytes;
	const uint64_t off_model = off_labels + label_bytes;
	const uint64_t off_codes = off_model + stored_model.size();
	const uint64_t off_tail = off_codes + cr.total;
	const uint64_t total = off_tail + 4ull * (sz + 1);
	uint8_t* o;
	if (early.p && total <= early_cap) { o = static_cast<uint8_t*>(early.p); early.p = nullptr; }
	else {
		o = static_cast<uint8_t*>(host_out_alloc(total));
		if (early.p && label_bytes) memcpy(o + off_labels, static_cast<uint8_t*>(early.p) + off_labels, label_bytes);
	}
	try {
		e.last_codes_total = cr.total;
		if (head.label_format == PINS_VARIABLE_WIDTH) {
			if (label_bytes) memcpy(o + off_labels, pins_binary.data(), label_bytes);
			labels_crc = crc32c(o + off_labels, label_bytes);
		}
		std::vector<uint8_t> hb;
		head.write(hb);
		memcpy(o, hb.data(), hb.size());
		auto put4 = [&](uint64_t at, uint32_t v) { for (int b = 0; b < 4; b++) o[at + b] = static_cast<uint8_t>((v >> (8 * b)) & 0xFF); };
		for (int64_t z = 0; z < sz; z++) put4(off_index + 4ull * z, cr.code_len[z]);
		put4(off_index + 4ull * sz, crc32c(o + off_index, 4ull * sz));
		if (!stored_model.empty()) memcpy(o + off_model, stored_model.data(), stored_model.size());
		for (int64_t z = 0; z < sz; z++) put4(off_tail + 4 + 4ull * z, fr.crcs[z]);
		put4(off_tail, labels_crc);
		e.device_stream_bytes = 0;
		if (e.keep_device_stream) {
			e.d_stream_out.ensure(total + 16);
			uint8_t* ds = e.d_stream_out.p;
			const void* up = head.label_format == FLAT ? o : nullptr;
			upload_small(ds, o, off_labels, s, up);
			if (label_bytes) {
				if (head.label_format == FLAT) copy_bytes_device(e.d_labels_bin.p, ds + off_labels, label_bytes, s);
				else CKL_HIP(hipMemcpyAsync(ds + off_labels, o + off_labels, label_bytes, hipMemcpyHostToDevice, s));
			}
			if (!stored_model.empty()) upload_small(ds + off_model, o + off_model, stored_model.size(), s, up);
			if (cr.total) copy_bytes_device(e.d_codes_out.p, ds + off_codes, cr.total, s);
			upload_small(ds + off_tail, o + off_tail, 4ull * (sz + 1), s, up);
			if (labels_stay) {
				CKL_HIP(hipStreamWaitEvent(s, e.ev_labels_crc, 0));
				CKL_HIP(hipMemcpyAsync(ds + off_tail, e.d_labels_crc.p, 4, hipMemcpyDeviceToDevice, s));
			}
			e.device_stream_bytes = total;
		}
		if (cr.total && !e.defer_codes) {
			if (e.async_host_copy && e.keep_device_stream) {
				if (!e.stream_copy) CKL_HIP(hipStreamCreateWithFlags(&e.stream_copy, hipStreamNonBlocking));
				if (!e.ev_codes) CKL_HIP(hipEventCreateWithFlags(&e.ev_codes, hipEventDisableTiming));
				CKL_HIP(hipEventRecord(e.ev_codes, s));
				CKL_HIP(hipStreamWaitEvent(e.stream_copy, e.ev_codes, 0));
				CKL_HIP(hipMemcpyAsync(o + off_codes, e.d_codes_out.p, cr.total, hipMemcpyDeviceToHost, e.stream_copy));
				if (labels_stay) {
					CKL_HIP(hipMemcpyAsync(o + off_labels, e.d_labels_bin.p, label_bytes, hipMemcpyDeviceToHost, e.stream_copy));
					CKL_HIP(hipMemcpyAsync(o + off_tail, e.d_labels_crc.p, 4, hipMemcpyDeviceToHost, e.stream_copy));
				}
				e.host_copy_pending = true;
			}
			else CKL_HIP(hipMemcpyAsync(o + off_codes, e.d_codes_out.p, cr.total, hipMemcpyDeviceToHost, s));
		}
		ht.mark("assembly");
		CKL_HIP(hipEventRecord(e.ev1, s));
		CKL_HIP(hipStreamSynchronize(s));
		ht.mark("codes_d2h");
		CKL_HIP(hipGetLastError());
		CKL_HIP(hipEventElapsedTime(&e.pipeline_ms, e.ev0, e.ev1));
		CKL_HIP(hipEventElapsedTime(&e.dominant_ms, e.evd0, e.evd1));
	}
	catch (...) {
		drain_host_copy(e, true);
		host_out_free(o);
		throw;
	}
	if (e.label_src) e.host_marks = ht.marks;
	*out = o;
	*out_len = total;
}

}

void ckl::encode_from_planes(
	ckl_encoder& e, const RunLabels& labels, int64_t sx, int64_t sy, int64_t sz, int data_width, bool fortran_order,
	uint64_t markov_model_order, const VolumeStats& st, const std::vector<uint32_t>& counts, uint8_t** out, uint64_t* out_len
) {
	planes_adopt_counts(e, counts, static_cast<uint32_t>(sz));
	e.planes_stats = st;
	e.planes_deferred = false;
	e.planes_dims[0] = sx; e.planes_dims[1] = sy; e.planes_dims[2] = sz;
	struct Source {
		ckl_encoder& e;
		Source(ckl_encoder& enc, const RunLabels* l) : e(enc) { e.label_src = l; e.planes_for = l; }
		~Source() { e.label_src = nullptr; e.planes_for = nullptr; }
	} source(e, &labels);
	const EncodeRequest req = { false, fortran_order, markov_model_order };
	with_label_type(data_width, [&](auto t) { encode_typed<typename decltype(t)::type>(e, nullptr, sx, sy, sz, req, out, out_len); });
}

namespace {

void reencode_markov(const uint8_t* buf, uint64_t n, int markov_order, int device, uint8_t** out, uint64_t* out_len) {
	if (n < Header::kBytesV0) throw Error(CKL_ERR_FORMAT, "crackle: Input too small to be a valid stream. Bytes: " + std::to_string(n));
	Header head = Header::parse(buf, n);
	if (markov_order < 0 || markov_order > 13) throw Error(CKL_ERR_ARG, "crackle_amd: markov_model_order must be in [0, 13] on device");
	if (head.markov_model_order == markov_order) { hand_out(buf, n, OutAlloc::HOST_OUT, out, out_len); return; }
	const bool v0 = head.format_version == 0;
	const uint64_t sz = head.sz;
	const uint64_t tail_bytes = v0 ? 0 : 4 * (sz + 1);
	const uint64_t off_index = head.header_bytes();
	const uint64_t off_labels = off_index + head.grid_index_bytes();
	if (!head.layout_fits(n)) throw Error(CKL_ERR_RUNTIME, "crackle: get_crack_code_offsets: Unable to read past end of buffer.");
	const uint64_t old_codes = off_labels + head.num_label_bytes + head.markov_model_bytes();
	uint64_t old_tail = old_codes;
	for (uint64_t z = 0; z < sz; z++) old_tail += rd_le(buf + off_index + 4 * z, 4);
	if (old_tail > n || tail_bytes > n - old_tail) throw Error(CKL_ERR_RUNTIME, "crackle: get_crack_codes: Unable to read past end of buffer.");

	const bool prof = getenv("CKL_PROFILE") != nullptr;
	auto t_prev = std::chrono::steady_clock::now();
	auto lap = [&](const char* what) {
		if (!prof) return;
		const auto now = std::chrono::steady_clock::now();
		fprintf(stderr, "[ckl reencode host ms] %s=%.2f\n", what, std::chrono::duration<double, std::milli>(now - t_prev).count());
		t_prev = now;
	};
	struct DecoderGuard { ckl_decoder* d = nullptr; ~DecoderGuard() { if (d) ckl_decoder_destroy(d); } } dec;
	struct EncoderGuard { ckl_encoder* e = nullptr; ~EncoderGuard() { if (e) ckl_encoder_destroy(e); } } enc;
	if (ckl_decoder_create(buf, n, 0, -1, device, &dec.d) != CKL_OK) throw Error(CKL_ERR_RUNTIME, ckl_last_error());
	lap("decoder_create");
	CrackResult cr;
	std::vector<uint8_t> stored_model;
	head.markov_model_order = markov_order;
	if (head.voxels() > 0) {
		const uint32_t *cv = nullptr, *ch = nullptr;
		uint32_t row_words = 0;
		uint64_t plane_words = 0;
		if (ckl_decoder_crack_planes(dec.d, &cv, &ch, &row_words, &plane_words) != CKL_OK) throw Error(CKL_ERR_RUNTIME, ckl_last_error());
		lap("crack_planes");
		if (ckl_encoder_create(head.sx, head.sy, head.sz, 1, device, &enc.e) != CKL_OK) throw Error(CKL_ERR_RUNTIME, ckl_last_error());
		lap("encoder_create");
		ckl_encoder& e = *enc.e;
		hipStream_t s = e.stream;
		const uint32_t ns = head.sz;
		const bool permissible = head.crack_format == PERMISSIBLE;
		planes_adopt(e, row_words, plane_words, ns, 2);
		hipLaunchKernelGGL(k_planes_from_cracks, dim3(static_cast<uint32_t>((plane_words + kBlock - 1) / kBlock), ns), dim3(kBlock), 0, s,
			cv, ch, head.sx, head.sy, row_words, plane_words, permissible ? 1u : 0u,
			plane_v(e), plane_h(e, ns), e.d_count_vh.p, ns);
// ... 193 lines not shown
			crq.markov_order = static_cast<int>(markov_model_order);
			const bool cached = planes_cached(*e, labels_device, sx, sy, sz);
			if (!cached) planes_pass_any(*e, labels_device, sx, sy, sz, nullptr);
			e->trail_for = nullptr;
			graph_pass(*e, sx, sy, sz, graph_format(crq.permissible));
			h = crack_pass(*e, sx, sy, sz, crq).hist;
			if (cached) { e->trail_for = labels_device; e->trail_perm = crq.permissible; e->trail_order = crq.markov_order; }
		}
		memcpy(hist, h.data(), h.size() * sizeof(uint32_t));
	});
}

static uint32_t* encoder_components(ckl_encoder* e, const void* labels_device, int64_t sx, int64_t sy, int64_t sz, uint32_t id_base, uint32_t* cc_device, uint32_t* ncomp_host) {
	check_dims(sx, sy, sz, e->dtype_bytes, 0);
	enter(e);
	const uint64_t voxels = static_cast<uint64_t>(sx) * sy * sz;
	if (voxels == 0) return cc_device;
	FlatResult fr;
	if (!planes_cached(*e, labels_device, sx, sy, sz)) planes_pass_any(*e, labels_device, sx, sy, sz, nullptr);
	flat_enqueue(*e, labels_device, sx, sy, sz, true, false);
	with_label_type(e->dtype_bytes, [&](auto t) { flat_collect(*e, static_cast<const typename decltype(t)::type*>(labels_device), sx, sy, sz, fr); });
	if (fr.total + id_base > 0xFFFFFFFFull) throw Error(CKL_ERR_RUNTIME, "crackle_amd: too many components");
	hipStream_t s2 = e->stream2;
	if (!cc_device) { e->d_cc_volume.ensure(voxels); cc_device = e->d_cc_volume.p; }
	launch_paint_components(s2, plane_v(*e), e->row_words, e->plane_words, sx, sy, sz, e->d_word_base.p, e->d_rbase.p, e->d_run_cc.p, e->d_comp_off.p, id_base, cc_device);
	for (int64_t z = 0; z < sz; z++) ncomp_host[z] = fr.ncomp[z];
	return cc_device;
}

int ckl_encoder_components(
	ckl_encoder* e, const void* labels_device, int64_t sx, int64_t sy, int64_t sz,
	uint32_t id_base, uint32_t* cc_host, uint32_t* ncomp_host
) {
	return guard([&] {
		if (!e || !cc_host || !ncomp_host) throw Error(CKL_ERR_ARG, "crackle_amd: null argument");
		const uint32_t* cc = encoder_components(e, labels_device, sx, sy, sz, id_base, nullptr, ncomp_host);
		const uint64_t voxels = static_cast<uint64_t>(sx) * sy * sz;
		if (voxels) CKL_HIP(hipMemcpyAsync(cc_host, cc, voxels * sizeof(uint32_t), hipMemcpyDeviceToHost, e->stream2));
		CKL_HIP(hipStreamSynchronize(e->stream2));
	});
}

int ckl_encoder_components_device(
	ckl_encoder* e, const void* labels_device, int64_t sx, int64_t sy, int64_t sz,
	uint32_t id_base, uint32_t* cc_device, uint32_t* ncomp_host
) {
	return guard([&] {
		if (!e || !cc_device || !ncomp_host) throw Error(CKL_ERR_ARG, "crackle_amd: null argument");
		encoder_components(e, labels_device, sx, sy, sz, id_base, cc_device, ncomp_host);
		CKL_HIP(hipStreamSynchronize(e->stream2));
	});
}

int ckl_encoder_last_timing(const ckl_encoder* e, float* pipeline_ms, float* dominant_kernel_ms) {
	if (!e) { set_last_error("crackle_amd: null encoder"); return CKL_ERR_ARG; }
	if (pipeline_ms) *pipeline_ms = e->pipeline_ms;
	if (dominant_kernel_ms) *dominant_kernel_ms = e->dominant_ms;
	return CKL_OK;
}

int ckl_encoder_walk_paths(ckl_encoder* e, uint32_t* fast_slices, uint32_t* compiled_slices) {
	return guard([&] {
		if (!e) throw Error(CKL_ERR_ARG, "crackle_amd: null encoder");
		uint32_t fast = 0, plain = 0;
		const size_t ns = e->last_trail_slices;
		if (ns && e->t_counters.p) {
			select_device(e->device);
			std::vector<uint32_t> nev(ns);
			CKL_HIP(hipMemcpy(nev.data(), e->t_counters.p + 5 * ns, ns * sizeof(uint32_t), hipMemcpyDeviceToHost));
			for (uint32_t v : nev) { if (v & (kEvFormatAddr12 | kEvWalkWide)) fast++; else if (v) plain++; }
		}
		if (fast_slices) *fast_slices = fast;
		if (compiled_slices) *compiled_slices = plain;
	});
}

int ckl_encoder_emit_path(const ckl_encoder* e, int* fused, uint64_t* lds_bytes) {
	if (!e) { set_last_error("crackle_amd: null encoder"); return CKL_ERR_ARG; }
	if (fused) *fused = e->emit_fused ? 1 : 0;
	if (lds_bytes) *lds_bytes = e->emit_lds;
	return CKL_OK;
}

int ckl_encoder_walk_step_kinds(ckl_encoder* e, uint32_t* counts, uint32_t max_slices, uint32_t* n_slices) {
	return guard([&] {
		if (!e || !counts || !n_slices) throw Error(CKL_ERR_ARG, "crackle_amd: null argument");
		const size_t ns = e->last_trail_slices;
		*n_slices = static_cast<uint32_t>(ns);
		if (!ns || !e->t_counters.p || !e->t_events.p) { *n_slices = 0; return; }
		if (ns > max_slices) throw Error(CKL_ERR_ARG, "crackle_amd: counts holds fewer slices than the last run had");
		select_device(e->device);
		DevBuf<uint32_t> d_counts;
		d_counts.ensure(ns * 5);
		hipLaunchKernelGGL(k_trail_step_kinds, dim3(static_cast<uint32_t>(ns)), dim3(kBlock), 0, e->stream, e->t_events.p, e->t_ibase.p, e->t_counters.p + 5 * ns, d_counts.p);
		CKL_HIP(hipMemcpyAsync(counts, d_counts.p, ns * 5 * sizeof(uint32_t), hipMemcpyDeviceToHost, e->stream));
		CKL_HIP(hipStreamSynchronize(e->stream));
	});
}

void ckl_encoder_destroy(ckl_encoder* e) { delete e; }

int ckl_compress(
	const void* labels, int labels_mem, int dtype_bytes, int is_signed,
	int64_t sx, int64_t sy, int64_t sz,
	int allow_pins, int fortran_order, uint64_t markov_model_order,
	int optimize_pins, int auto_bgcolor, int64_t manual_bgcolor,
	int device, uint8_t** out, uint64_t* out_len
) {
	ckl_encoder* e = nullptr;
	try {
		check_dims(sx, sy, sz, dtype_bytes, is_signed);
		if (!out || !out_len) throw Error(CKL_ERR_ARG, "crackle_amd: null argument");
		if (static_cast<uint64_t>(sx) * sy * sz == 0) {
			hand_out(header_bytes(stream_header(dtype_bytes, sx, sy, sz, VolumeStats(), allow_pins != 0, fortran_order != 0, markov_model_order, nullptr)), OutAlloc::MALLOC, out, out_len);
			return CKL_OK;
		}
	}
	catch (const Error& err) { set_last_error(err.what()); return err.status; }
	const int rc = ckl_encoder_create(sx, sy, sz, dtype_bytes, device, &e);
	if (rc != CKL_OK) return rc;
	const EncoderPtr owner(e);
	return guard([&]() -> int {
		const uint64_t bytes = static_cast<uint64_t>(sx) * sy * sz * dtype_bytes;
		const void* dev_labels = labels;
		DevBuf<uint8_t> tmp;
		if (labels_mem == CKL_MEM_HOST && bytes) {
			if (!labels) throw Error(CKL_ERR_ARG, "crackle_amd: null labels");
			tmp.ensure(bytes);
			CKL_HIP(hipMemcpy(tmp.p, labels, bytes, hipMemcpyHostToDevice));
			dev_labels = tmp.p;
		}
		return ckl_encoder_run(e, dev_labels, sx, sy, sz, allow_pins, fortran_order, markov_model_order,
			optimize_pins, auto_bgcolor, manual_bgcolor, nullptr, out, out_len);
	});
}

}
```

crackle_amd/csrc/ckl_encoder.hpp:

```cpp
#pragma once

#include "ckl_common.hpp"

#include <chrono>
#include <utility>

struct VolumeStats { uint64_t max_label = 0, pairs = 0, first = 0, last = 0; };
namespace ckl { namespace dev { struct RunLabels; } }

struct ckl_encoder {
	template <typename T> using DevBuf = ckl::DevBuf<T>;

	int device = 0;
	hipStream_t stream = nullptr;
	hipStream_t stream2 = nullptr;
	hipEvent_t ev0 = nullptr, ev1 = nullptr, ev_in = nullptr;
	hipEvent_t evd0 = nullptr, evd1 = nullptr;
	hipEvent_t ev_prezero = nullptr;
	float pipeline_ms = 0.f, dominant_ms = 0.f;
	int dtype_bytes = 0;

	DevBuf<unsigned long long> d_stats;
	DevBuf<uint4> d_adjm;
	DevBuf<uint32_t> d_slice_err;
	DevBuf<uint64_t> d_cbase, d_sbase, d_kbase, d_pbase, d_bbase, d_out_off, d_comp_off;
	DevBuf<uint32_t> d_ccap, d_scap, d_kcap;
	DevBuf<uint8_t> d_crack_tables;
	DevBuf<uint8_t> d_cp, d_fcode, d_dcode, d_payload, d_boc, d_codes_out, d_model;
	DevBuf<uint32_t> d_code_report;
	uint64_t codes_capacity = 0;
	bool defer_codes = false;
	bool keep_device_stream = false;
	bool async_host_copy = false;
	bool host_copy_pending = false;
	hipStream_t stream_copy = nullptr;
	hipStream_t stream_tab = nullptr;
	hipEvent_t ev_codes = nullptr;
	void* tables_staging = nullptr;
	bool uploads_by_kernel = false;
	hipEvent_t ev_labels_crc = nullptr;
	DevBuf<uint32_t> d_labels_crc;
	DevBuf<uint8_t> d_stream_out;
	uint64_t device_stream_bytes = 0;
	uint64_t last_codes_total = 0;
	DevBuf<uint32_t> d_stack_node, d_stack_code;
	DevBuf<uint32_t> d_chain_node, d_chain_off, d_chain_clen, d_chain_order, d_chain_dst, d_chain_vstart;
	DevBuf<uint32_t> d_n_chains, d_n_raw, d_n_valid, d_payload_len, d_boc_len;
	DevBuf<uint32_t> d_hist;
	DevBuf<uint32_t> d_planes, d_count_vh;
	uint32_t row_words = 0;
	uint64_t plane_words = 0;
	std::vector<uint32_t> count_v, count_h;
	DevBuf<uint64_t> d_rbase;
	DevBuf<uint32_t> d_rcap, d_word_base, d_parent, d_run_start, d_run_cc, d_comp_pix, d_nruns, d_ncomp, d_idbits, d_blk_roots;
	DevBuf<uint16_t> d_run_local;
	DevBuf<uint32_t> d_G, d_crc_acc;
	DevBuf<uint32_t> d_flat_report;
	uint64_t g_table_pixels = 0;
	DevBuf<uint64_t> d_mapping, d_sorted, d_uniq, d_label_hash, d_label_list;
	DevBuf<uint32_t> d_cc_volume;
	DevBuf<uint32_t> d_pin_kept, d_pin_u32;
	DevBuf<uint8_t> d_pin_tables;
	DevBuf<uint64_t> d_pin_u64;
	DevBuf<uint32_t> d_slice_err2, d_n_uniq, d_uniq_blk;
	DevBuf<uint8_t> d_labels_bin;
	const void* planes_for = nullptr;
	const void* trail_for = nullptr;
	bool trail_perm = false;
	int trail_order = 0;
	const ckl::dev::RunLabels* label_src = nullptr;
	std::vector<std::pair<const char*, double>> host_marks;
	VolumeStats planes_stats;
	int64_t planes_dims[3] = { 0, 0, 0 };
	std::vector<uint64_t> h_rbase;
	std::vector<uint32_t> h_rcap;
	std::vector<uint64_t> h_comp_off;
	DevBuf<uint16_t> s_run_lid, s_seam_first, s_seam_last;
	DevBuf<uint32_t> s_sc_w, s_sc_first, s_strip_nruns, s_strip_nsc;
	DevBuf<uint64_t> d_label_slots;
	uint32_t flat_nstrips = 0, flat_strip_rows = 0, flat_strip_cap = 0, flat_resolve_cap = 0;
	int max_lds = 0;
	bool flat_strips = false;
	std::vector<uint32_t> count_special, count_corner;
	DevBuf<uint32_t> d_plane_partial, t_blk_special, t_blk_corner;
	DevBuf<unsigned long long> d_plane_partial_max, d_plane_out;
	uint32_t graph_blocks = 0;
	uint32_t tiles_x = 0, tiles_y = 0, mtx2 = 0;
	uint64_t adjm_stride = 0;
	bool graph_permissible = false;
	bool planes_deferred = false;
	bool trail_zeroed = false;
	DevBuf<uint64_t> t_nbase, t_cobase, t_ibase;
	DevBuf<uint32_t> t_ncap, t_cocap, t_icap, t_max_steps;
	bool emit_fused = false;
	size_t emit_lds = 0;
	size_t last_trail_slices = 0;
	DevBuf<uint32_t> t_counters;
	DevBuf<uint32_t> t_node_vertex, t_vert2node, t_corner_vertex;
	DevBuf<uint8_t> t_node_adj;
	DevBuf<uint32_t> t_dart_end, t_dart_len, t_dart_minv, t_dart_minpos, t_parent, t_start_bits, t_starts;
	DevBuf<uint4> t_dart_codes;
	DevBuf<uint8_t> t_dart_inline;
	DevBuf<unsigned long long> t_compmin;
	DevBuf<uint32_t> t_items, t_item_off, t_chain_item0, t_events, t_chain_ev0, t_ev_lnd, t_ev_item;

	~ckl_encoder() {
		if (ev0) (void)hipEventDestroy(ev0);
		if (ev1) (void)hipEventDestroy(ev1);
		if (evd0) (void)hipEventDestroy(evd0);
		if (evd1) (void)hipEventDestroy(evd1);
		if (ev_in) (void)hipEventDestroy(ev_in);
		if (ev_prezero) (void)hipEventDestroy(ev_prezero);
		if (stream) (void)hipStreamDestroy(stream);
		if (stream2) (void)hipStreamDestroy(stream2);
		if (stream_copy) { (void)hipStreamSynchronize(stream_copy); (void)hipStreamDestroy(stream_copy); }
		if (stream_tab) { (void)hipStreamSynchronize(stream_tab); (void)hipStreamDestroy(stream_tab); }
		if (ev_codes) (void)hipEventDestroy(ev_codes);
		if (tables_staging) ckl::host_out_free(tables_staging);
		if (ev_labels_crc) (void)hipEventDestroy(ev_labels_crc);
	}
};

namespace ckl {

template <typename T>
inline std::vector<T> download(const T* p, size_t n, hipStream_t s) {
	std::vector<T> h(n);
	if (n) CKL_HIP(hipMemcpyAsync(h.data(), p, n * sizeof(T), hipMemcpyDeviceToHost, s));
	CKL_HIP(hipStreamSynchronize(s));
	return h;
}

struct HostTimer {
	bool on;
	std::chrono::steady_clock::time_point t0;
	std::vector<std::pair<const char*, double>> marks;
	HostTimer() : on(getenv("CKL_PROFILE") != nullptr), t0(std::chrono::steady_clock::now()) {}
	void mark(const char* name) {
		if (!on) return;
		auto t1 = std::chrono::steady_clock::now();
		marks.emplace_back(name, std::chrono::duration<double, std::milli>(t1 - t0).count());
		t0 = t1;
	}
	~HostTimer();
};
inline thread_local HostTimer* g_ht = nullptr;
#define HT_MARK(name) do { if (g_ht) g_ht->mark(name); } while (0)
inline HostTimer::~HostTimer() {
		g_ht = nullptr;
		if (!on) return;
		fprintf(stderr, "[ckl encode host ms]");
		for (auto& m : marks) fprintf(stderr, " %s=%.2f", m.first, m.second);
		fprintf(stderr, "\n");
}

inline void enter(ckl_encoder* e) {
	if (!e) throw Error(CKL_ERR_ARG, "crackle_amd: null encoder");
	select_device(e->device);
	wait_for_default_stream(e->stream, e->ev_in);
	wait_for_default_stream(e->stream2, e->ev_in);
}

inline void drain_host_copy(ckl_encoder& e, bool quiet = false) {
	if (!e.host_copy_pending) return;
	if (quiet) (void)hipStreamSynchronize(e.stream_copy);
	else CKL_HIP(hipStreamSynchronize(e.stream_copy));
	e.host_copy_pending = false;
}

enum class OutAlloc { MALLOC, HOST_OUT };
inline void hand_out(const uint8_t* bytes, size_t n, OutAlloc how, uint8_t** out, uint64_t* out_len) {
	uint8_t* p = static_cast<uint8_t*>(how == OutAlloc::MALLOC ? malloc(n ? n : 1) : host_out_alloc(n ? n : 1));
	if (!p) throw Error(CKL_ERR_RUNTIME, "crackle_amd: out of host memory");
	if (n) memcpy(p, bytes, n);
	*out = p;
	*out_len = n;
}
inline void hand_out(const std::vector<uint8_t>& bin, OutAlloc how, uint8_t** out, uint64_t* out_len) { hand_out(bin.data(), bin.size(), how, out, out_len); }

inline uint32_t* plane_v(const ckl_encoder& e) { return e.d_planes.p; }
inline uint32_t* plane_h(const ckl_encoder& e, uint32_t ns) { return e.d_planes.p + e.plane_words * ns; }

void check_dims(int64_t sx, int64_t sy, int64_t sz, int dtype_bytes, int is_signed);
Header stream_header(int data_width, int64_t sx, int64_t sy, int64_t sz, const VolumeStats& st, bool allow_pins, bool fortran_order, uint64_t markov_model_order, const ckl_encode_overrides* ov);
inline std::vector<uint8_t> header_bytes(const Header& head) {
	std::vector<uint8_t> hb;
	head.write(hb);
	return hb;
}

void planes_adopt(ckl_encoder& e, uint32_t row_words, uint64_t plane_words, uint32_t ns, uint32_t count_rows);
void planes_adopt_counts(ckl_encoder& e, const std::vector<uint32_t>& counts, uint32_t ns);
void encode_from_planes(
	ckl_encoder& e, const dev::RunLabels& labels, int64_t sx, int64_t sy, int64_t sz, int data_width, bool fortran_order,
	uint64_t markov_model_order, const VolumeStats& st, const std::vector<uint32_t>& counts, uint8_t** out, uint64_t* out_len);

template <typename LABEL>
std::vector<uint8_t> pins_section_plain(
	ckl_encoder& e, const LABEL* labels, const uint32_t* cc, const uint64_t* comp_label, int64_t sx, int64_t sy, int64_t sz, uint64_t N,
	const std::vector<uint32_t>& nc, int index_width, int stored_width, bool auto_bgcolor, int64_t manual_bgcolor);

}
// ... 1 lines not shown
```

crackle_amd/csrc/ckl_trail.hpp:

```cpp
#pragma once

#include "ckl_device.hpp"

namespace ckl {
namespace dev {

constexpr uint32_t kTrailTileShift = 5, kTrailTileDim = 32;
__device__ __forceinline__ uint32_t mt_index(uint32_t mx, uint32_t my, uint32_t mtx2) {
	return (((my >> 1) * mtx2 + (mx >> 1)) << 2) | ((my & 1u) << 1) | (mx & 1u);
}
struct MicroTile {
	uint4 lo, hi;
	uint32_t mx, my;
	__device__ __forceinline__ bool holds(uint32_t x, uint32_t y) const { return (x >> 3) == mx && (y >> 3) == my; }
	__device__ __forceinline__ uint32_t nib(uint32_t x, uint32_t y) const {
		const uint32_t r = y & 7u;
		const uint32_t a0 = (r & 1u) ? lo.y : lo.x, a1 = (r & 1u) ? lo.w : lo.z, a2 = (r & 1u) ? hi.y : hi.x, a3 = (r & 1u) ? hi.w : hi.z;
		const uint32_t b0 = (r & 2u) ? a1 : a0, b1 = (r & 2u) ? a3 : a2;
		return (((r & 4u) ? b1 : b0) >> ((x & 7u) * 4u)) & 15u;
	}
};

enum : uint32_t { TRAIL_ERR_CAPACITY = 1u };
constexpr uint32_t kDartNone = 0xFFFFFFFFu;
constexpr uint32_t kItemSeg = 0u << 30, kItemCtl = 1u << 30, kItemDead = 2u << 30, kItemMask = 3u << 30;

struct TrailArgs {
	const uint4* adjm;
	uint64_t adjm_stride;
	uint32_t mtx2;
	uint32_t tiles_x, tiles_y;
	const uint32_t* planeV;
	const uint32_t* planeH;
	uint32_t row_words;
	uint64_t plane_words;
	uint32_t sx, sy, inv;
	uint32_t sxe, sye;
	uint32_t nverts;
	uint32_t z0;
	const uint32_t* max_steps;
	uint32_t graph_blocks;
	const uint32_t* blk_special;
	const uint32_t* blk_corner;
	const uint64_t* nbase;
	const uint32_t* ncap;
	uint32_t* n_nodes;
	uint32_t* node_vertex;
	uint8_t* node_adj;
	uint32_t* vert2node;
	const uint64_t* cobase;
	const uint32_t* cocap;
	uint32_t* n_corners;
	uint32_t* corner_vertex;
	uint32_t* dart_end;
	uint32_t* dart_len;
	uint32_t* dart_minv;
	uint32_t* dart_minpos;
	uint4* dart_codes;
	uint8_t* dart_inline;
	uint32_t* parent;
	unsigned long long* compmin;
	uint32_t* start_bits;
	uint32_t start_words;
	uint32_t* starts;
	uint32_t* n_starts;
	const uint64_t* ibase;
	const uint32_t* icap;
	uint32_t* items;
	uint32_t* item_off;
	uint32_t* n_items;
	const uint64_t* sbase;
	const uint32_t* scap;
	uint32_t* stack_node;
	uint32_t* stack_item;
	const uint64_t* kbase;
	const uint32_t* kcap;
	uint32_t* chain_node;
	uint32_t* chain_item0;
	uint32_t* chain_off;
	uint32_t* chain_clen;
	uint32_t* n_chains;
	uint32_t* n_raw;
	uint32_t* n_valid;
	const uint64_t* cbase;
	const uint32_t* ccap;
	uint8_t* cp;
	uint32_t* slice_err;
	uint32_t* events;
	uint32_t* n_events;
	uint32_t* seg_len_sum;
	uint32_t* chain_ev0;
	uint32_t* ev_lnd;
	uint32_t* ev_item;
	uint32_t walk_plain;
	uint32_t walk_stack_cap;
	uint32_t walk_no_regs;
	unsigned long long* dbg;
};

__device__ __forceinline__ void mt_load(MicroTile& c, const uint4* adjm, uint32_t x, uint32_t y, uint32_t mtx2) {
	const uint4* p = adjm + static_cast<uint64_t>(mt_index(x >> 3, y >> 3, mtx2)) * 2u;
	c.lo = p[0]; c.hi = p[1];
	c.mx = x >> 3; c.my = y >> 3;
}
__device__ __forceinline__ void trail_step(uint32_t& x, uint32_t& y, uint32_t k) {
	if (k & 2u) y = (k & 1u) ? y - 1u : y + 1u;
// ... 54 lines not shown
	uint32_t hw[8], hpw[8], vw[9];
#pragma unroll
	for (uint32_t k = 0; k < 8; k++) {
		const uint64_t row = static_cast<uint64_t>(min(y0 + k, sy - 1u)) * row_words;
		hw[k] = ph[row + txc];
		hpw[k] = ph[row + txp];
	}
#pragma unroll
	for (uint32_t k = 0; k < 9; k++) {
		const uint32_t y = y0 + k;
		vw[k] = pv[static_cast<uint64_t>(min(y > 0 ? y - 1u : 0u, sy - 1u)) * row_words + txc];
	}
#pragma unroll
	for (uint32_t k = 0; k < 8; k++) {
		const uint32_t y = y0 + k;
		const uint32_t h = have_w ? hw[k] : 0u, hp = tx > 0 ? hpw[k] : 0u;
		if (y >= 1 && y < sy) {
			b[k].R = (h ^ inv) & lt_sx;
			b[k].L = (((h << 1) | (hp >> 31)) ^ inv) & ge_1 & le_sx;
		}
		if (y < sy) b[k].D = ((have_w ? vw[k + 1] : 0u) ^ inv) & ge_1 & lt_sx;
		if (y >= 1 && y <= sy) b[k].U = ((have_w ? vw[k] : 0u) ^ inv) & ge_1 & lt_sx;
	}
}

static __global__ void __launch_bounds__(kBlock) k_trail_graph(
	const uint32_t* __restrict__ planeV, const uint32_t* __restrict__ planeH, uint32_t row_words, uint64_t plane_words,
	uint32_t sx, uint32_t sy, uint32_t perm_mode, const unsigned long long* __restrict__ total_pairs, unsigned long long half_voxels,
	uint32_t* __restrict__ adjm_words, uint64_t adjm_stride_words,
	uint32_t mtx2, uint32_t tiles_x, uint32_t tiles_y, uint32_t* __restrict__ blk_special, uint32_t* __restrict__ blk_corner
) {
	__shared__ uint32_t s_red[2 * kWaves];
	__shared__ uint4 s_out[kWaves][kWave * 8];
	const int lane = threadIdx.x & 63, wave = threadIdx.x >> 6;
	const uint32_t zi = blockIdx.y;
	const bool permissible = perm_mode == 2u ? static_cast<long long>(*total_pairs) < static_cast<long long>(half_voxels) : perm_mode != 0u;
	const uint32_t item = blockIdx.x * kBlock + threadIdx.x;
	const uint32_t mtx = (sx + 1u + 7u) >> 3;
	uint32_t ns = 0, nc = 0;
	uint32_t my_base = 0, my_tiles = 0;
	if (item < tiles_x * tiles_y) {
		const uint32_t ty = item / tiles_x, tx = item - ty * tiles_x;
		TileRowBits b[8];
		trail_rows8(planeV + zi * plane_words, planeH + zi * plane_words, row_words, sx, sy, tx, ty << 3, permissible ? 0xFFFFFFFFu : 0u, b);
		my_base = mt_index(tx * 4u, ty, mtx2) * 32u;
		my_tiles = min(4u, mtx - min(mtx, tx * 4u));
#pragma unroll
		for (uint32_t q = 0; q < 4; q++) {
			uint32_t w[8];
#pragma unroll
			for (uint32_t k = 0; k < 8; k++)
				w[k] = spread8((b[k].R >> (8 * q)) & 255u) | (spread8((b[k].L >> (8 * q)) & 255u) << 1)
					| (spread8((b[k].D >> (8 * q)) & 255u) << 2) | (spread8((b[k].U >> (8 * q)) & 255u) << 3);
			s_out[wave][lane * 8 + ((2u * q) ^ (lane & 7))] = make_uint4(w[0], w[1], w[2], w[3]);
			s_out[wave][lane * 8 + ((2u * q + 1u) ^ (lane & 7))] = make_uint4(w[4], w[5], w[6], w[7]);
		}
#pragma unroll
		for (uint32_t k = 0; k < 8; k++) { ns += __popc(trail_special_mask(b[k])); nc += __popc(trail_corner_mask(b[k])); }
	}
	{
		uint8_t* dst = reinterpret_cast<uint8_t*>(adjm_words + zi * adjm_stride_words);
#pragma unroll
		for (uint32_t i = 0; i < 8; i++) {
			const uint32_t owner = i * 8u + (lane >> 3), p = lane & 7u;
			const uint32_t base = __shfl(my_base, owner, kWave), have = __shfl(my_tiles, owner, kWave);
			const uint4 v = s_out[wave][owner * 8u + (p ^ (owner & 7u))];
			const uint32_t q = p >> 1;
			if (q < have) *reinterpret_cast<uint4*>(dst + base + (q >> 1) * 128u + (q & 1u) * 32u + (p & 1u) * 16u) = v;
		}
	}
	ns = wave_sum(ns); nc = wave_sum(nc);
	if (lane == 0) { s_red[wave] = ns; s_red[kWaves + wave] = nc; }
	__syncthreads();
	if (threadIdx.x == 0) {
		uint32_t ts = 0, tc = 0;
		for (int w = 0; w < kWaves; w++) { ts += s_red[w]; tc += s_red[kWaves + w]; }
		blk_special[static_cast<uint64_t>(zi) * gridDim.x + blockIdx.x] = ts;
		blk_corner[static_cast<uint64_t>(zi) * gridDim.x + blockIdx.x] = tc;
	}
}

static __global__ void __launch_bounds__(kBlock) k_trail_count_scan(
	uint32_t* __restrict__ blk_special, uint32_t* __restrict__ blk_corner, uint32_t nblk,
	uint32_t* __restrict__ tot_special, uint32_t* __restrict__ tot_corner
) {
	__shared__ uint32_t s_scan[2 * kWaves];
	const uint32_t zi = blockIdx.x;
	uint32_t* bs = blk_special + static_cast<uint64_t>(zi) * nblk;
	uint32_t* bc = blk_corner + static_cast<uint64_t>(zi) * nblk;
	uint32_t cs = 0, cc = 0;
	for (uint32_t b0 = 0; b0 < nblk; b0 += kBlock) {
		const uint32_t b = b0 + threadIdx.x;
		uint32_t v[2] = { b < nblk ? bs[b] : 0u, b < nblk ? bc[b] : 0u }, tot[2];
		block_excl_add<2>(v, tot, s_scan);
		if (b < nblk) { bs[b] = cs + v[0]; bc[b] = cc + v[1]; }
		cs += tot[0]; cc += tot[1];
	}
	if (threadIdx.x == 0) { tot_special[zi] = cs; tot_corner[zi] = cc; }
}

static __global__ void __launch_bounds__(kBlock) k_trail_nodes(TrailArgs a) {
	__shared__ uint32_t s_scan[2 * kWaves];
	const uint32_t zi = blockIdx.y + a.z0;
	const uint32_t item = blockIdx.x * kBlock + threadIdx.x;
	TileRowBits b[8];
	uint32_t x0 = 0, y0 = 0;
	if (item < a.tiles_x * a.tiles_y) {
		const uint32_t ty = item / a.tiles_x, tx = item - ty * a.tiles_x;
		x0 = tx << kTrailTileShift; y0 = ty << 3;
		trail_rows8(a.planeV + zi * a.plane_words, a.planeH + zi * a.plane_words, a.row_words, a.sx, a.sy, tx, y0, a.inv, b);
	}
	else {
#pragma unroll
		for (int k = 0; k < 8; k++) b[k] = TileRowBits{ 0, 0, 0, 0 };
	}
	uint32_t v[2] = { 0, 0 }, tot[2];
#pragma unroll
	for (uint32_t k = 0; k < 8; k++) { v[0] += __popc(trail_special_mask(b[k])); v[1] += __popc(trail_corner_mask(b[k])); }
	block_excl_add<2>(v, tot, s_scan);
	uint32_t j = a.blk_special[static_cast<uint64_t>(zi) * a.graph_blocks + blockIdx.x] + v[0];
	uint32_t c = a.blk_corner[static_cast<uint64_t>(zi) * a.graph_blocks + blockIdx.x] + v[1];
	const uint64_t nb = a.nbase[zi];
	const uint32_t ncap = a.ncap[zi], cocap = a.cocap[zi];
	uint32_t err = 0;
#pragma unroll
	for (uint32_t k = 0; k < 8; k++) {
		const uint32_t y = y0 + k;
		const TileRowBits& r = b[k];
		for (uint32_t m = trail_special_mask(r); m; m &= m - 1u) {
			const uint32_t i = __ffs(m) - 1;
			const uint32_t vtx = y * a.sxe + x0 + i;
			if (j < ncap) {
				a.node_vertex[nb + j] = vtx;
				a.node_adj[nb + j] = static_cast<uint8_t>(((r.R >> i) & 1u) | (((r.L >> i) & 1u) << 1) | (((r.D >> i) & 1u) << 2) | (((r.U >> i) & 1u) << 3));
				a.vert2node[static_cast<uint64_t>(zi) * a.nverts + vtx] = j;
			}
			else err = TRAIL_ERR_CAPACITY;
			j++;
		}
		for (uint32_t m = trail_corner_mask(r); m; m &= m - 1u) {
			const uint32_t i = __ffs(m) - 1;
			if (c < cocap) a.corner_vertex[a.cobase[zi] + c] = y * a.sxe + x0 + i;
			else err = TRAIL_ERR_CAPACITY;
			c++;
		}
	}
	if (err) atomicOr(a.slice_err + zi, err);
	if (blockIdx.x == gridDim.x - 1 && threadIdx.x == kBlock - 1) {
		a.n_nodes[zi] = min(j, ncap);
		a.n_corners[zi] = min(c, cocap);
	}
}

constexpr uint32_t kWalkChunk = 192;
constexpr uint32_t kExpandChunk = 384;
constexpr int kWalkRefill = 8;
constexpr int kWalkAhead = 2;
constexpr uint32_t kInlineCodes = 64;

static __global__ void __launch_bounds__(kBlock) k_trail_segments(TrailArgs a) {
	__shared__ uint4 s_res[kWaves][kWalkChunk];
	__shared__ uint4 s_codes[kWaves][kWalkChunk];
	const uint32_t zi = blockIdx.y + a.z0;
	const uint32_t lane = threadIdx.x & (kWave - 1);
	const uint32_t wv = threadIdx.x >> 6;
	const uint32_t wave = blockIdx.x * kWaves + wv;
	const uint32_t n_darts = min(a.n_nodes[zi], a.ncap[zi]) * 4u;
	const uint32_t range_begin = wave * kWalkChunk;
	uint32_t next = range_begin;
	const uint32_t range_end = min(next + kWalkChunk, n_darts);
	if (next >= range_end) return;
	const uint64_t nb = a.nbase[zi];
	const uint4* adjm = a.adjm + zi * a.adjm_stride;
	const uint32_t* v2n = a.vert2node + static_cast<uint64_t>(zi) * a.nverts;
	const uint32_t cap = a.max_steps[zi];
	const unsigned long long lt_mask = (1ull << lane) - 1ull;
	uint4* res = s_res[wv];
	uint4* res_codes = s_codes[wv];
	for (uint32_t i = lane; i < kWalkChunk; i += kWave) res[i] = make_uint4(kDartNone, 0u, 0u, 0u);
	MicroTile c;
	c.lo = c.hi = make_uint4(0, 0, 0, 0); c.mx = c.my = 0xFFFFFFFFu;
// ... 1336 lines not shown
```

include/crackle_amd.h:

```cpp
#ifndef CRACKLE_AMD_H
#define CRACKLE_AMD_H

#include <stdint.h>

#ifdef __cplusplus
extern "C" {
#endif

typedef enum ckl_status {
	CKL_OK = 0,
	CKL_ERR_FORMAT = 1,
	CKL_ERR_RUNTIME = 2,
	CKL_ERR_ARG = 3,
	CKL_ERR_NO_DEVICE = 4,
	CKL_ERR_CRC = 5
} ckl_status;

enum { CKL_MEM_HOST = 0, CKL_MEM_DEVICE = 1 };

const char* ckl_last_error(void);

int ckl_abi_version(void);

int ckl_device_count(void);
// ... 72 lines not shown
                       void* out_device, uint64_t out_capacity_bytes, int has_label, uint64_t label);
int ckl_cutout(const uint8_t* buf, uint64_t n, void* out, uint64_t out_capacity_bytes, int out_mem,
               int64_t x0, int64_t x1, int64_t y0, int64_t y1, int64_t z0, int64_t z1,
               int has_label, uint64_t label, int device);
int ckl_paste(const uint8_t* buf, uint64_t n,
              const void* box, int box_mem, int has_box, uint64_t value,
              int64_t x0, int64_t x1, int64_t y0, int64_t y1, int64_t z0, int64_t z1,
              int device, uint8_t** out, uint64_t* out_len);
int ckl_decoder_last_timing(const ckl_decoder* d, float* pipeline_ms, float* dominant_kernel_ms);
int ckl_decoder_stage_timing(const ckl_decoder* d, int index, const char** name, float* ms);
int ckl_decoder_set_stage_events(ckl_decoder* d, int on);
void ckl_decoder_destroy(ckl_decoder* d);

typedef struct ckl_encoder ckl_encoder;

int ckl_encoder_create(int64_t sx, int64_t sy, int64_t sz, int dtype_bytes, int device, ckl_encoder** out);

typedef struct ckl_encode_overrides {
	int32_t force_crack_format;
	int32_t force_label_format;
	int32_t force_stored_width;
	int32_t has_model;
	const uint8_t* model;
	int (*merge_unique)(void* ctx, const uint64_t* local_distinct, uint64_t n_local,
	                    const uint64_t** merged_sorted, uint64_t* n_merged);
	void* merge_ctx;
} ckl_encode_overrides;

int ckl_encoder_run(
	ckl_encoder* e, const void* labels_device,
	int64_t sx, int64_t sy, int64_t sz,
	int allow_pins, int fortran_order, uint64_t markov_model_order,
	int optimize_pins, int auto_bgcolor, int64_t manual_bgcolor,
	const ckl_encode_overrides* overrides,
	uint8_t** out, uint64_t* out_len);

int ckl_encoder_defer_codes(ckl_encoder* e, int defer);
int ckl_encoder_keep_device_stream(ckl_encoder* e, int keep);
int ckl_encoder_async_host_copy(ckl_encoder* e, int on);
int ckl_encoder_host_wait(ckl_encoder* e);
int ckl_encoder_device_stream(const ckl_encoder* e, const uint8_t** stream_device, uint64_t* n_bytes);
int ckl_encoder_codes_to_host(ckl_encoder* e, uint8_t* dst_host, uint64_t capacity, uint64_t* n_bytes);
int ckl_host_register(void* p, uint64_t bytes);
int ckl_host_unregister(void* p);

int ckl_encoder_stats(
	ckl_encoder* e, const void* labels_device, int64_t sx, int64_t sy, int64_t sz,
	uint64_t* max_label, uint64_t* pixel_pairs, uint64_t* first_voxel, uint64_t* last_voxel);

int ckl_encoder_markov_stats(
	ckl_encoder* e, const void* labels_device, int64_t sx, int64_t sy, int64_t sz,
	int crack_format, uint64_t markov_model_order, uint32_t* hist);

int ckl_encoder_components(
	ckl_encoder* e, const void* labels_device, int64_t sx, int64_t sy, int64_t sz,
	uint32_t id_base, uint32_t* cc_host, uint32_t* ncomp_host);

int ckl_encoder_components_device(
	ckl_encoder* e, const void* labels_device, int64_t sx, int64_t sy, int64_t sz,
	uint32_t id_base, uint32_t* cc_device, uint32_t* ncomp_host);

int ckl_encoder_pin_labels(
	ckl_encoder* e, const void* labels_device, const uint32_t* cc_device,
	int64_t sx, int64_t sy, int64_t sz, const uint32_t* ncomp_host,
	int stored_width, int auto_bgcolor, int64_t manual_bgcolor,
	uint8_t** out, uint64_t* out_len);

int ckl_pins_rows_first(ckl_encoder* e, const void* labels_rows, const uint32_t* cc_rows, int64_t sx, int64_t rows, int64_t sz, int64_t y0,
	uint64_t n_components, uint64_t* first_any, uint64_t* first_kept, uint64_t* comp_label);
int ckl_pins_rows_best(ckl_encoder* e, const void* labels_rows, const uint32_t* cc_rows, int64_t sx, int64_t rows, int64_t sz, int64_t y0,
	uint64_t n_components, const uint64_t* first_kept, uint64_t* best);
int ckl_pins_rows_extent(ckl_encoder* e, const void* labels_rows, const uint32_t* cc_rows, int64_t sx, int64_t rows, int64_t sz, int64_t y0,
	uint64_t n_components, const uint64_t* first_kept, const uint64_t* best, uint64_t* choice, uint32_t* ze_plus1);
int ckl_pins_rows_ids(ckl_encoder* e, const uint32_t* cc_rows, int64_t sx, int64_t rows, int64_t sz, int64_t y0,
	uint64_t n_components, const uint64_t* choice, const uint32_t* ze_plus1, const uint64_t* offsets, uint32_t* ids);
int ckl_pins_rows_section(ckl_encoder* e, int64_t sx, int64_t sy, int64_t sz, uint64_t n_components, const uint32_t* ncomp_host,
	const uint64_t* comp_label, const uint64_t* first_any, const uint64_t* choice, const uint32_t* ze_plus1, const uint64_t* offsets, const uint32_t* ids,
	int stored_width, int auto_bgcolor, int64_t manual_bgcolor, uint8_t** out, uint64_t* out_len);

int ckl_encoder_last_timing(const ckl_encoder* e, float* pipeline_ms, float* dominant_kernel_ms);
int ckl_encoder_walk_paths(ckl_encoder* e, uint32_t* fast_slices, uint32_t* compiled_slices);
int ckl_encoder_emit_path(const ckl_encoder* e, int* fused, uint64_t* lds_bytes);
int ckl_encoder_walk_step_kinds(ckl_encoder* e, uint32_t* counts, uint32_t max_slices, uint32_t* n_slices);
void ckl_encoder_destroy(ckl_encoder* e);


int ckl_zstack(
	const uint8_t* const* bufs, const uint64_t* lens, uint64_t count,
	uint8_t** out, uint64_t* out_len);

int ckl_pin_labels_host(
	const void* labels, int dtype_bytes, const uint32_t* cc,
	int64_t sx, int64_t sy, int64_t sz, const uint32_t* ncomp,
	int stored_width, int auto_bgcolor, int64_t manual_bgcolor,
	uint8_t** out, uint64_t* out_len);

int ckl_point_cloud(
	const uint8_t* buf, uint64_t n, int64_t z_start, int64_t z_end,
	const uint64_t* labels, uint64_t n_labels, int has_labels, int skip_background, int device,
	uint64_t** labels_out, uint64_t** offsets_out, uint16_t** points_out, uint64_t* n_out);

int ckl_reencode_markov(const uint8_t* buf, uint64_t n, int markov_model_order, int device, uint8_t** out, uint64_t* out_len);

int ckl_recompress(const uint8_t* buf, uint64_t n, int markov_model_order, int device, uint8_t** out, uint64_t* out_len);

#define CKL_ERODE_KEEP_BORDER 1
int ckl_erode(const uint8_t* buf, uint64_t n, int connectivity, int flags, int markov_model_order, int device,
              uint8_t** out, uint64_t* out_len);

int ckl_dilate(const uint8_t* buf, uint64_t n, int connectivity, int flags, int markov_model_order, int device,
               uint8_t** out, uint64_t* out_len);

int ckl_zsplit(const uint8_t* buf, uint64_t n, int64_t z_start, int64_t z_end, uint8_t** out, uint64_t* out_len);

int ckl_connected_components(
	const uint8_t* buf, uint64_t n, int connectivity, int device,
	uint8_t** out, uint64_t* out_len, uint64_t** component_labels, uint64_t* n_components);

int ckl_relabel_components(const uint8_t* buf, uint64_t n, const uint64_t* new_ids, uint64_t n_ids, uint8_t** out, uint64_t* out_len);

#define CKL_DUST_BINARY_IMAGE 1
#define CKL_DUST_INVERT       2
int ckl_dust(const uint8_t* buf, uint64_t n, uint64_t threshold, int connectivity, int flags, int device,
             uint8_t** out, uint64_t* out_len, uint64_t* n_removed );

int ckl_fill_holes(const uint8_t* buf, uint64_t n, int connectivity, int device,
                   uint8_t** out, uint64_t* out_len, uint64_t* n_filled );

int ckl_relabel_values(const uint8_t* buf, uint64_t n, const uint64_t* values, uint64_t n_values,
                       uint8_t** out, uint64_t* out_len);

uint32_t ckl_crc32c(const uint8_t* data, uint64_t n);
uint32_t ckl_crc32c_combine(uint32_t crc_a, uint32_t crc_b, uint64_t len_b);

#ifdef __cplusplus
}
#endif
#endif
```

Baseline: 167.6 billion.

## Count trail nodes in plane kernel and seal output stream on device

The label-plane kernel now also counts special and corner trail nodes per slice. This lets the host size the trail buffers early from a side stream instead of waiting for the count-scan download, and the count-scan kernel checks the early counts against its own and flags any mismatch. A device-side seal assembles the header, index, CRC and tail of the final stream with kernels, so the final host synchronize can be skipped. Small device-to-host reads go through a pinned staging buffer written by a kernel. These changes add LDS use and work in the plane kernel and more code-path complexity, with risks to correctness at boundaries.

```diff
diff --git a/crackle_amd/_lib.py b/crackle_amd/_lib.py
--- a/crackle_amd/_lib.py
+++ b/crackle_amd/_lib.py
@@ -98,6 +98,7 @@
   "ckl_encoder_last_timing": (C.c_int, [C.c_void_p, C.POINTER(C.c_float), C.POINTER(C.c_float)]),
   "ckl_encoder_walk_paths": (C.c_int, [C.c_void_p, C.POINTER(C.c_uint32), C.POINTER(C.c_uint32)]),
   "ckl_encoder_emit_path": (C.c_int, [C.c_void_p, C.POINTER(C.c_int), C.POINTER(C.c_uint64)]),
+  "ckl_encoder_node_counts": (C.c_int, [C.c_void_p, C.POINTER(C.c_uint32), C.c_uint32, C.POINTER(C.c_uint32), C.POINTER(C.c_int), C.POINTER(C.c_int)]),
   "ckl_encoder_destroy": (None, [C.c_void_p]),
   "ckl_pin_labels_host": (C.c_int, [
     C.c_void_p, C.c_int, C.c_void_p, C.c_int64, C.c_int64, C.c_int64, C.c_void_p,
diff --git a/crackle_amd/csrc/ckl_encode.hip b/crackle_amd/csrc/ckl_encode.hip
--- a/crackle_amd/csrc/ckl_encode.hip
+++ b/crackle_amd/csrc/ckl_encode.hip
@@ -138,20 +138,22 @@
 __global__ void __launch_bounds__(kBlock) k_label_planes_stream(
 	const LABEL* __restrict__ labels, uint32_t sx, uint32_t sy, uint32_t strips, uint32_t bands,
 	uint32_t* __restrict__ planeV, uint32_t* __restrict__ planeH, uint32_t row_words, uint64_t plane_words,
-	uint32_t* __restrict__ partial, unsigned long long* __restrict__ partial_max, unsigned long long* __restrict__ total_pairs
+	uint32_t* __restrict__ partial, uint32_t* __restrict__ partial_nodes ,
+	unsigned long long* __restrict__ partial_max, unsigned long long* __restrict__ total_pairs
 ) {
 	if (blockIdx.x == 0 && blockIdx.y == 0 && threadIdx.x == 0) *total_pairs = 0;
 	constexpr uint32_t P = 16 / sizeof(LABEL);
 	constexpr uint32_t G = 32 / P;
 	constexpr uint32_t WPR = 64 / G;
 	struct alignas(16) Vec { LABEL v[P]; };
-	__shared__ uint32_t s_red[3 * kWaves];
+	__shared__ uint32_t s_red[5 * kWaves];
 	__shared__ unsigned long long s_max[kWaves];
 	__shared__ __attribute__((aligned(16))) uint32_t s_words[kWaves][2][kBandRows * WPR];
+	__shared__ uint32_t s_vprev[kWaves][WPR];
 	const uint32_t zi = blockIdx.y;
 	const uint32_t lane = threadIdx.x & 63u, wave = threadIdx.x >> 6;
 	const uint32_t task = blockIdx.x * kWaves + wave;
-	uint32_t nv = 0, nh = 0, pairs = 0;
+	uint32_t nv = 0, nh = 0, pairs = 0, nspecial = 0, ncorner = 0;
 	LABEL mxl = 0;
 	if (task < strips * bands) {
 		const uint32_t band = __builtin_amdgcn_readfirstlane(task / strips), strip = __builtin_amdgcn_readfirstlane(task - (task / strips) * strips);
@@ -189,6 +191,25 @@
 		};
 #pragma unroll
 		for (uint32_t r = 0; r < kRowsAhead; r++) request(r, y0 + r);
+		LABEL edge_above = 0;
+		uint32_t h_left = 0;
+		{
+			bool have_above = false;
+			uint32_t bv = 0;
+			if (y0 > 0) {
+				edge_above = edge_of(y0 - 1u, have_above);
+				LABEL left = wave_shift_up1_label(prev.v[P - 1]);
+				if (lane == 0) left = edge_above;
+				if (active) {
+#pragma unroll
+					for (uint32_t i = 0; i < P; i++) bv |= (prev.v[i] != (i ? prev.v[i - 1] : left) ? 1u : 0u) << i;
+					if (x == 0) bv &= ~1u;
+				}
+			}
+			bv <<= (lane % G) * P;
+			bv = or_over_lane_group<G>(bv);
+			if ((lane % G) == 0) s_vprev[wave][lane / G] = bv;
+		}
 #pragma unroll
 		for (uint32_t it = 0; it < kBandRows / kRowsAhead; it++) {
 			const uint32_t yb = y0 + it * kRowsAhead;
@@ -200,6 +221,8 @@
 				const bool have_edge = have_edges[r];
 				request(r, y + kRowsAhead);
 				if (y >= y1) continue;
+				if (x0 > 0 && y > 0 && edge != edge_above) h_left |= 1u << (y - y0);
+				edge_above = edge;
 				LABEL left = wave_shift_up1_label(cur.v[P - 1]);
 				bool have_left = true;
 				if (lane == 0) { left = edge; have_left = have_edge; }
@@ -240,18 +263,35 @@
 				for (uint32_t q = 0; q < kVecWords; q++) if (word0 + w + q < row_words) { pv[at + q] = sv[r * WPR + w + q]; ph[at + q] = sh[r * WPR + w + q]; }
 			}
 		}
-	}
-	nv = wave_sum(nv); nh = wave_sum(nh); pairs = wave_sum(pairs);
+		{
+			const uint32_t nrows = y1 - y0;
+			const bool column_sx = x0 + 64u * P == sx;
+			for (uint32_t i = lane; i < nrows * WPR; i += kWave) {
+				const uint32_t r = i / WPR, w = i % WPR;
+				const uint32_t h = sh[r * WPR + w];
+				dev::TileRowBits b;
+				b.R = h;
+				b.L = (h << 1) | (w ? sh[r * WPR + w - 1] >> 31 : (h_left >> r) & 1u);
+				b.D = sv[r * WPR + w];
+				b.U = r ? sv[(r - 1u) * WPR + w] : s_vprev[wave][w];
+				nspecial += __popc(dev::trail_special_mask(b)) + ((column_sx && w == WPR - 1u) ? h >> 31 : 0u);
+				ncorner += __popc(dev::trail_corner_mask(b));
+				if (y1 == sy && r == nrows - 1u) nspecial += __popc(b.D);
+			}
+		}
+	}
+	nv = wave_sum(nv); nh = wave_sum(nh); pairs = wave_sum(pairs); nspecial = wave_sum(nspecial); ncorner = wave_sum(ncorner);
 	unsigned long long mx = static_cast<unsigned long long>(mxl);
 	for (int d = kWave / 2; d >= 1; d >>= 1) { const unsigned long long o = __shfl_xor(mx, d, kWave); mx = o > mx ? o : mx; }
-	if (lane == 0) { s_red[wave] = nv; s_red[kWaves + wave] = nh; s_red[2 * kWaves + wave] = pairs; s_max[wave] = mx; }
+	if (lane == 0) { s_red[wave] = nv; s_red[kWaves + wave] = nh; s_red[2 * kWaves + wave] = pairs; s_red[3 * kWaves + wave] = nspecial; s_red[4 * kWaves + wave] = ncorner; s_max[wave] = mx; }
 	__syncthreads();
 	if (threadIdx.x == 0) {
-		uint32_t tv = 0, th = 0, tp = 0;
+		uint32_t tv = 0, th = 0, tp = 0, ts = 0, tc = 0;
 		unsigned long long tm = 0;
-		for (int w = 0; w < kWaves; w++) { tv += s_red[w]; th += s_red[kWaves + w]; tp += s_red[2 * kWaves + w]; tm = s_max[w] > tm ? s_max[w] : tm; }
+		for (int w = 0; w < kWaves; w++) { tv += s_red[w]; th += s_red[kWaves + w]; tp += s_red[2 * kWaves + w]; ts += s_red[3 * kWaves + w]; tc += s_red[4 * kWaves + w]; tm = s_max[w] > tm ? s_max[w] : tm; }
 		const uint64_t o = static_cast<uint64_t>(zi) * gridDim.x + blockIdx.x;
 		partial[o * 4 + 0] = tv; partial[o * 4 + 1] = th; partial[o * 4 + 2] = tp; partial[o * 4 + 3] = 0;
+		partial_nodes[o * 2 + 0] = ts; partial_nodes[o * 2 + 1] = tc;
 		partial_max[o] = tm;
 	}
 }
@@ -286,28 +326,31 @@
 }
 
 __global__ void __launch_bounds__(kBlock) k_planes_reduce(
-	const uint32_t* __restrict__ partial, const unsigned long long* __restrict__ partial_max, uint32_t nblk,
+	const uint32_t* __restrict__ partial, const uint32_t* __restrict__ partial_nodes, const unsigned long long* __restrict__ partial_max, uint32_t nblk,
 	unsigned long long* __restrict__ out ,
-	unsigned long long* __restrict__ total_pairs
+	unsigned long long* __restrict__ total_pairs ,
+	unsigned long long* __restrict__ out_nodes
 ) {
 	__shared__ uint32_t s_red[kWaves];
 	__shared__ unsigned long long s_max[kWaves];
 	const uint32_t zi = blockIdx.x;
-	uint32_t tv = 0, th = 0, tp = 0;
+	uint32_t tv = 0, th = 0, tp = 0, ts = 0, tc = 0;
 	unsigned long long tm = 0;
 	for (uint32_t b = threadIdx.x; b < nblk; b += kBlock) {
 		const uint64_t o = static_cast<uint64_t>(zi) * nblk + b;
 		tv += partial[o * 4 + 0]; th += partial[o * 4 + 1]; tp += partial[o * 4 + 2];
+		ts += partial_nodes[o * 2 + 0]; tc += partial_nodes[o * 2 + 1];
 		const unsigned long long m = partial_max[o];
 		tm = m > tm ? m : tm;
 	}
-	tv = block_sum(tv, s_red); th = block_sum(th, s_red); tp = block_sum(tp, s_red);
+	tv = block_sum(tv, s_red); th = block_sum(th, s_red); tp = block_sum(tp, s_red); ts = block_sum(ts, s_red); tc = block_sum(tc, s_red);
 	for (int d = kWave / 2; d >= 1; d >>= 1) { const unsigned long long o = __shfl_xor(tm, d, kWave); tm = o > tm ? o : tm; }
 	if ((threadIdx.x & 63) == 0) s_max[threadIdx.x >> 6] = tm;
 	__syncthreads();
 	if (threadIdx.x == 0) {
 		for (int w = 0; w < kWaves; w++) tm = s_max[w] > tm ? s_max[w] : tm;
 		out[4ull * zi + 0] = tv; out[4ull * zi + 1] = th; out[4ull * zi + 2] = tp; out[4ull * zi + 3] = tm;
+		out_nodes[2ull * zi + 0] = ts; out_nodes[2ull * zi + 1] = tc;
 		atomicAdd(total_pairs, static_cast<unsigned long long>(tp));
 	}
 }
@@ -1217,7 +1260,7 @@
 	if (threadIdx.x == 0) out[0] = ~(s_st[0] ^ init_term);
 }
 
-__global__ void __launch_bounds__(kBlock) k_copy_bytes(const uint8_t* __restrict__ src, uint8_t* __restrict__ dst, uint64_t n) {
+__device__ __forceinline__ void copy_bytes_body(const uint8_t* __restrict__ src, uint8_t* __restrict__ dst, uint64_t n) {
 	const uint64_t head = min(n, static_cast<uint64_t>((4u - (reinterpret_cast<uintptr_t>(dst) & 3u)) & 3u));
 	const uint64_t words = (n - head) / 4u;
 	const uint64_t tid = static_cast<uint64_t>(blockIdx.x) * kBlock + threadIdx.x;
@@ -1235,6 +1278,42 @@
 	else {
 		for (uint64_t i = tid; i < words; i += stride) dw[i] = __funnelshift_r(sw[i], sw[i + 1], sh);
 	}
+}
+__global__ void __launch_bounds__(kBlock) k_copy_bytes(const uint8_t* __restrict__ src, uint8_t* __restrict__ dst, uint64_t n) { copy_bytes_body(src, dst, n); }
+
+__device__ __forceinline__ uint64_t report_total(const uint32_t* __restrict__ report, uint32_t nslices) {
+	return static_cast<uint64_t>(report[nslices]) | (static_cast<uint64_t>(report[nslices + 1]) << 32);
+}
+__global__ void __launch_bounds__(kBlock) k_copy_bytes_reported(
+	const uint8_t* __restrict__ src, uint8_t* __restrict__ dst, const uint32_t* __restrict__ report, uint32_t nslices, uint64_t cap
+) {
+	const uint64_t n = report_total(report, nslices);
+	if (n <= cap) copy_bytes_body(src, dst, n);
+}
+__global__ void __launch_bounds__(kBlock) k_words_to_host(const uint32_t* __restrict__ src, uint32_t* __restrict__ dst_host, uint32_t n) {
+	const uint32_t i = blockIdx.x * kBlock + threadIdx.x;
+	if (i < n) dst_host[i] = src[i];
+}
+__global__ void __launch_bounds__(kBlock) k_stream_index(const uint32_t* __restrict__ report, uint32_t nslices, uint32_t* __restrict__ index_words) {
+	const uint32_t z = blockIdx.x * kBlock + threadIdx.x;
+	if (z < nslices) index_words[z] = report[z];
+}
+__global__ void __launch_bounds__(kBlock) k_stream_tail(
+	const uint32_t* __restrict__ report, uint32_t nslices, const uint32_t* __restrict__ index_words, const uint32_t* __restrict__ index_crc,
+	const uint8_t* __restrict__ header, uint32_t header_bytes, const uint32_t* __restrict__ tail, const uint32_t* __restrict__ labels_crc,
+	uint8_t* __restrict__ stream, uint8_t* __restrict__ codes, uint64_t cap
+) {
+	const uint32_t i = blockIdx.x * kBlock + threadIdx.x;
+	if (i < header_bytes) stream[i] = header[i];
+	if (i > nslices) return;
+	const uint32_t iv = i < nslices ? index_words[i] : *index_crc;
+	uint8_t* ip = stream + header_bytes + 4ull * i;
+	for (uint32_t b = 0; b < 4; b++) ip[b] = static_cast<uint8_t>(iv >> (8u * b));
+	const uint64_t total = report_total(report, nslices);
+	if (total > cap) return;
+	const uint32_t tv = (i == 0u && labels_crc) ? *labels_crc : tail[i];
+	uint8_t* tp = codes + total + 4ull * i;
+	for (uint32_t b = 0; b < 4; b++) tp[b] = static_cast<uint8_t>(tv >> (8u * b));
 }
 
 __global__ void __launch_bounds__(kBlock) k_trail_step_kinds(const uint32_t* __restrict__ events, const uint64_t* __restrict__ ibase, const uint32_t* __restrict__ n_events, uint32_t* __restrict__ counts) {
@@ -1346,17 +1425,48 @@
 	return permissible ? interior - differ : differ;
 }
 
-void planes_collect(ckl_encoder& e, uint32_t ns, VolumeStats* st, const std::vector<unsigned long long>* fetched = nullptr) {
+void* staging_block(ckl_encoder& e, size_t bytes) {
+	if (e.report_staging_bytes < bytes) {
+		if (e.report_staging) host_out_free(e.report_staging);
+		e.report_staging = nullptr; e.report_staging_bytes = 0;
+		const size_t cap = std::max<size_t>(bytes, 64u << 10);
+		e.report_staging = host_out_alloc(cap);
+		e.report_staging_bytes = cap;
+	}
+	return e.report_staging;
+}
+
+const uint32_t* fetch_words(ckl_encoder& e, const void* src, size_t n, hipStream_t s) {
+	uint32_t* dst = static_cast<uint32_t*>(staging_block(e, n * sizeof(uint32_t)));
+	if (host_out_is_pinned(dst) && n <= (1u << 20)) hipLaunchKernelGGL(k_words_to_host, dim3(static_cast<uint32_t>((n + kBlock - 1) / kBlock)), dim3(kBlock), 0, s, static_cast<const uint32_t*>(src), dst, static_cast<uint32_t>(n));
+	else CKL_HIP(hipMemcpyAsync(dst, src, n * sizeof(uint32_t), hipMemcpyDeviceToHost, s));
+	return dst;
+}
+
+enum class EarlyCounts { ON, OFF, CHECK };
+inline EarlyCounts early_counts_mode() {
+	const char* env = getenv("CKL_EARLY_COUNTS");
+	if (!env) return EarlyCounts::ON;
+	if (!strcmp(env, "0")) return EarlyCounts::OFF;
+	return !strcmp(env, "check") ? EarlyCounts::CHECK : EarlyCounts::ON;
+}
+
+inline size_t plane_out_words(uint32_t ns) { return 6ull * ns + 1; }
+
+void planes_collect(ckl_encoder& e, uint32_t ns, VolumeStats* st, const unsigned long long* fetched = nullptr) {
 	std::vector<unsigned long long> mine;
-	if (!fetched) { mine = download(e.d_plane_out.p, 4ull * ns, e.stream); fetched = &mine; }
-	const std::vector<unsigned long long>& o = *fetched;
+	if (!fetched) { mine = download(e.d_plane_out.p, plane_out_words(ns), e.stream); fetched = mine.data(); }
+	const unsigned long long* o = fetched;
 	e.count_v.resize(ns); e.count_h.resize(ns);
+	e.early_special.resize(ns); e.early_corner.resize(ns);
 	VolumeStats v;
 	for (uint32_t zi = 0; zi < ns; zi++) {
 		e.count_v[zi] = static_cast<uint32_t>(o[4ull * zi]);
 		e.count_h[zi] = static_cast<uint32_t>(o[4ull * zi + 1]);
 		v.pairs += o[4ull * zi + 2];
 		v.max_label = std::max<uint64_t>(v.max_label, o[4ull * zi + 3]);
+		e.early_special[zi] = static_cast<uint32_t>(o[4ull * ns + 1 + 2ull * zi]);
+		e.early_corner[zi] = static_cast<uint32_t>(o[4ull * ns + 2 + 2ull * zi]);
 	}
 	e.planes_deferred = false;
 	if (st) *st = v;
@@ -1383,6 +1493,7 @@
 	const uint32_t ns = static_cast<uint32_t>(sz);
 	e.trail_zeroed = false;
 	e.planes_deferred = false;
+	e.early_counts = false;
 	e.row_words = static_cast<uint32_t>((sx + 31) / 32);
 	e.plane_words = static_cast<uint64_t>(e.row_words) * sy;
 	e.d_planes.ensure(2 * e.plane_words * ns);
@@ -1394,13 +1505,18 @@
 		const uint32_t nblk = (strips * bands + kWaves - 1) / kWaves;
 		e.d_plane_partial.ensure(4ull * nblk * ns);
 		e.d_plane_partial_max.ensure(static_cast<size_t>(nblk) * ns);
-		e.d_plane_out.ensure(4ull * ns + 1);
+		e.d_plane_partial_nodes.ensure(2ull * nblk * ns);
+		e.d_plane_out.ensure(plane_out_words(ns));
 		trail_prezero(e, sx, sy, sz);
 		hipLaunchKernelGGL(k_label_planes_stream<LABEL>, dim3(nblk, ns), dim3(kBlock), 0, s,
 			labels, static_cast<uint32_t>(sx), static_cast<uint32_t>(sy), strips, bands,
 			plane_v(e), plane_h(e, ns), e.row_words, e.plane_words,
-			e.d_plane_partial.p, e.d_plane_partial_max.p, e.d_plane_out.p + 4ull * ns);
-		hipLaunchKernelGGL(k_planes_reduce, dim3(ns), dim3(kBlock), 0, s, e.d_plane_partial.p, e.d_plane_partial_max.p, nblk, e.d_plane_out.p, e.d_plane_out.p + 4ull * ns);
+			e.d_plane_partial.p, e.d_plane_partial_nodes.p, e.d_plane_partial_max.p, e.d_plane_out.p + 4ull * ns);
+		hipLaunchKernelGGL(k_planes_reduce, dim3(ns), dim3(kBlock), 0, s, e.d_plane_partial.p, e.d_plane_partial_nodes.p, e.d_plane_partial_max.p, nblk,
+			e.d_plane_out.p, e.d_plane_out.p + 4ull * ns, e.d_plane_out.p + 4ull * ns + 1);
+		if (!e.ev_planes) CKL_HIP(hipEventCreateWithFlags(&e.ev_planes, hipEventDisableTiming));
+		CKL_HIP(hipEventRecord(e.ev_planes, s));
+		e.early_counts = true;
 		e.planes_deferred = defer;
 		if (!e.planes_deferred) planes_collect(e, ns, st);
 		return;
@@ -1447,20 +1563,52 @@
 		on_device ? e.d_plane_out.p + 4ull * ns : nullptr, half_voxels,
 		reinterpret_cast<uint32_t*>(e.d_adjm.p), e.adjm_stride * 4,
 		e.mtx2, e.tiles_x, e.tiles_y, e.t_blk_special.p, e.t_blk_corner.p);
+	const EarlyCounts mode = early_counts_mode();
+	const bool early = e.early_counts && mode == EarlyCounts::ON && format != GraphFormat::PERMISSIBLE;
+	if (early && e.trail_zeroed) CKL_HIP(hipStreamWaitEvent(s, e.ev_prezero, 0));
 	hipLaunchKernelGGL(k_trail_count_scan, dim3(ns), dim3(kBlock), 0, s, e.t_blk_special.p, e.t_blk_corner.p, e.graph_blocks,
-		e.d_count_vh.p + 2 * static_cast<size_t>(ns), e.d_count_vh.p + 3 * static_cast<size_t>(ns));
-	std::vector<unsigned long long> po;
-	if (e.planes_deferred) {
-		po.resize(4ull * ns);
+		e.d_count_vh.p + 2 * static_cast<size_t>(ns), e.d_count_vh.p + 3 * static_cast<size_t>(ns),
+		early && e.trail_zeroed ? e.d_plane_out.p + 4ull * ns + 1 : nullptr, static_cast<uint32_t>(format), on_device ? e.d_plane_out.p + 4ull * ns : nullptr, half_voxels,
+		e.d_slice_err.p);
+	const bool was_deferred = e.planes_deferred;
+	VolumeStats v;
+	bool counted = false;
+	e.early_counts_used = false;
+	if (was_deferred && early && e.trail_zeroed) {
+		if (!e.stream_copy) CKL_HIP(hipStreamCreateWithFlags(&e.stream_copy, hipStreamNonBlocking));
+		CKL_HIP(hipStreamWaitEvent(e.stream_copy, e.ev_planes, 0));
+		const unsigned long long* po = reinterpret_cast<const unsigned long long*>(fetch_words(e, e.d_plane_out.p, 2 * plane_out_words(ns), e.stream_copy));
+		CKL_HIP(hipStreamSynchronize(e.stream_copy));
+		planes_collect(e, ns, &v, po);
+	}
+	else if (was_deferred) {
+		std::vector<unsigned long long> po(plane_out_words(ns));
 		CKL_HIP(hipMemcpyAsync(po.data(), e.d_plane_out.p, po.size() * sizeof(unsigned long long), hipMemcpyDeviceToHost, s));
-	}
-	std::vector<uint32_t> c = download(e.d_count_vh.p + 2 * static_cast<size_t>(ns), 2 * static_cast<size_t>(ns), s);
-	e.count_special.assign(c.begin(), c.begin() + ns);
-	e.count_corner.assign(c.begin() + ns, c.end());
-	VolumeStats v;
-	if (!po.empty()) planes_collect(e, ns, &v, &po);
-	if (st && !po.empty()) *st = v;
+		std::vector<uint32_t> c = download(e.d_count_vh.p + 2 * static_cast<size_t>(ns), 2 * static_cast<size_t>(ns), s);
+		e.count_special.assign(c.begin(), c.begin() + ns);
+		e.count_corner.assign(c.begin() + ns, c.end());
+		counted = true;
+		planes_collect(e, ns, &v, po.data());
+	}
+	if (st && was_deferred) *st = v;
 	e.graph_permissible = on_device ? static_cast<int64_t>(v.pairs) < static_cast<int64_t>(static_cast<uint64_t>(sx) * sy * sz) / 2 : format == GraphFormat::PERMISSIBLE;
+	if (!counted && early && e.trail_zeroed && !e.graph_permissible) {
+		e.count_special = e.early_special;
+		e.count_corner = e.early_corner;
+		e.early_counts_used = true;
+		counted = true;
+	}
+	if (!counted) {
+		std::vector<uint32_t> c = download(e.d_count_vh.p + 2 * static_cast<size_t>(ns), 2 * static_cast<size_t>(ns), s);
+		e.count_special.assign(c.begin(), c.begin() + ns);
+		e.count_corner.assign(c.begin() + ns, c.end());
+	}
+	if (mode == EarlyCounts::CHECK && e.early_counts && !e.graph_permissible) {
+		for (uint32_t zi = 0; zi < ns; zi++)
+			if (e.early_special[zi] != e.count_special[zi] || e.early_corner[zi] != e.count_corner[zi])
+				throw Error(CKL_ERR_RUNTIME, "crackle_amd: node counts of the planes pass and of the graph differ on z=" + std::to_string(zi)
+					+ ": " + std::to_string(e.early_special[zi]) + " / " + std::to_string(e.early_corner[zi]) + " against " + std::to_string(e.count_special[zi]) + " / " + std::to_string(e.count_corner[zi]));
+	}
 }
 
 enum class CrackGoal { HISTOGRAM, CODES };
@@ -1471,6 +1619,8 @@
 	const std::vector<uint8_t>* model = nullptr;
 	bool reuse_trail = false;
 	std::function<void()> overlap;
+	std::function<void()> seal_index;
+	std::function<void()> seal;
 };
 struct CrackResult {
 	std::vector<uint32_t> code_len;
@@ -1581,7 +1731,10 @@
 
 void check_walk_errors(ckl_encoder& e, uint32_t ns) {
 	const std::vector<uint32_t> errs = download(e.d_slice_err.p, ns, e.stream);
-	for (uint32_t zi = 0; zi < ns; zi++) if (errs[zi]) throw Error(CKL_ERR_RUNTIME, "crackle_amd: crack walk scratch overflow on z=" + std::to_string(zi));
+	for (uint32_t zi = 0; zi < ns; zi++) {
+		if (errs[zi] & TRAIL_ERR_COUNTS) throw Error(CKL_ERR_RUNTIME, "crackle_amd: node counts of the planes pass and of the graph differ on z=" + std::to_string(zi));
+		if (errs[zi]) throw Error(CKL_ERR_RUNTIME, "crackle_amd: crack walk scratch overflow on z=" + std::to_string(zi));
+	}
 }
 
 CrackResult crack_pass(ckl_encoder& e, int64_t sx, int64_t sy, int64_t sz, const CrackRequest& rq) {
@@ -1741,6 +1894,7 @@
 			e.d_payload.p, e.d_pbase.p, e.d_payload_len.p, e.d_out_off.p, e.d_codes_out.p);
 	};
 	if (!markov_order) enqueue_tail();
+	if (!markov_order && rq.seal_index) rq.seal_index();
 	if (rq.overlap) rq.overlap();
 	HT_MARK("c:overlap");
 
@@ -1763,7 +1917,16 @@
 		enqueue_tail();
 	}
 	HT_MARK("c:finish_enq");
-	const std::vector<uint32_t> report = download(e.d_code_report.p, static_cast<size_t>(ns) + 3, s);
+	std::vector<uint32_t> report;
+	if (rq.seal && !markov_order) {
+		rq.seal();
+		const size_t words = static_cast<size_t>(ns) + 3;
+		const uint32_t* r = fetch_words(e, e.d_code_report.p, words, s);
+		CKL_HIP(hipEventRecord(e.ev1, s));
+		CKL_HIP(hipStreamSynchronize(s));
+		report.assign(r, r + words);
+	}
+	else report = download(e.d_code_report.p, static_cast<size_t>(ns) + 3, s);
 	HT_MARK("c:finish_wait");
 	if (report[ns + 2]) check_walk_errors(e, ns);
 	result.code_len.assign(report.begin(), report.begin() + ns);
@@ -2111,6 +2274,7 @@
 void ckl::planes_adopt(ckl_encoder& e, uint32_t row_words, uint64_t plane_words, uint32_t ns, uint32_t count_rows) {
 	e.row_words = row_words;
 	e.plane_words = plane_words;
+	e.early_counts = false;
 	e.d_planes.ensure(2 * plane_words * ns);
 	e.d_count_vh.ensure(4 * static_cast<size_t>(ns));
 	CKL_HIP(hipMemsetAsync(e.d_count_vh.p, 0, count_rows * static_cast<size_t>(ns) * sizeof(uint32_t), e.stream));
@@ -2260,8 +2424,52 @@
 		}
 	};
 
+	bool sealed = false;
+	auto seal_index = [&]() {
+		const uint32_t ns = static_cast<uint32_t>(sz);
+		e.d_seal_index.ensure(ns);
+		e.d_seal_crc.ensure(1 + kBlock);
+		hipLaunchKernelGGL(k_stream_index, dim3((ns + kBlock - 1) / kBlock), dim3(kBlock), 0, s, e.d_code_report.p, ns, e.d_seal_index.p);
+		crc32c_device(reinterpret_cast<const uint8_t*>(e.d_seal_index.p), 4ull * sz, e.d_seal_crc.p + 1, e.d_seal_crc.p, s);
+	};
+	auto seal = [&]() {
+		const uint32_t ns = static_cast<uint32_t>(sz);
+		const uint64_t off_codes = off_labels + label_bytes;
+		e.device_stream_bytes = 0;
+		e.d_stream_out.ensure(off_codes + e.codes_capacity + 4ull * (sz + 1) + 16);
+		uint8_t* ds = e.d_stream_out.p;
+		uint8_t* eo = static_cast<uint8_t*>(early.p);
+		head.num_label_bytes = label_bytes;
+		std::vector<uint8_t> hb;
+		head.write(hb);
+		memcpy(eo, hb.data(), hb.size());
+		uint32_t* stage = reinterpret_cast<uint32_t*>(eo + ((early_cap - 4ull * (sz + 1)) & ~15ull));
+		stage[0] = labels_crc;
+		for (int64_t z = 0; z < sz; z++) stage[1 + z] = fr.crcs[z];
+		const uint8_t* header_src = eo;
+		const uint32_t* tail_src = stage;
+		if (!host_out_is_pinned(eo)) {
+			e.d_seal_tail.ensure(static_cast<size_t>(ns) + 1 + 16);
+			upload_small(e.d_seal_tail.p, stage, 4ull * (sz + 1), s, nullptr);
+			upload_small(e.d_seal_tail.p + ns + 1, eo, hb.size(), s, nullptr);
+			tail_src = e.d_seal_tail.p;
+			header_src = reinterpret_cast<const uint8_t*>(e.d_seal_tail.p + ns + 1);
+		}
+		const uint32_t copy_blocks = static_cast<uint32_t>(std::min<uint64_t>((e.codes_capacity / 4u + kBlock - 1) / kBlock + 1u, 8192u));
+		hipLaunchKernelGGL(k_copy_bytes_reported, dim3(copy_blocks), dim3(kBlock), 0, s, e.d_codes_out.p, ds + off_codes, e.d_code_report.p, ns, e.codes_capacity);
+		if (labels_stay) CKL_HIP(hipStreamWaitEvent(s, e.ev_labels_crc, 0));
+		if (label_bytes) copy_bytes_device(e.d_labels_bin.p, ds + off_labels, label_bytes, s);
+		hipLaunchKernelGGL(k_stream_tail, dim3((ns + 1 + kBlock - 1) / kBlock), dim3(kBlock), 0, s, e.d_code_report.p, ns, e.d_seal_index.p, e.d_seal_crc.p,
+			header_src, static_cast<uint32_t>(hb.size()), tail_src, labels_stay ? e.d_labels_crc.p : nullptr, ds, ds + off_codes, e.codes_capacity);
+		sealed = true;
+	};
+
 	const bool no_overlap = getenv("CKL_NO_OVERLAP") != nullptr;
 	if (!no_overlap) crq.overlap = label_side;
+	{
+		const char* sw = getenv("CKL_DEVICE_SEAL");
+		if (!no_overlap && !(sw && !strcmp(sw, "0")) && head.label_format == FLAT && head.markov_model_order == 0 && e.keep_device_stream && !e.defer_codes) { crq.seal_index = seal_index; crq.seal = seal; }
+	}
 	const CrackResult cr = crack_pass(e, sx, sy, sz, crq);
 	if (no_overlap) label_side();
 	ht.mark("cracks");
@@ -2295,7 +2503,8 @@
 		for (int64_t z = 0; z < sz; z++) put4(off_tail + 4 + 4ull * z, fr.crcs[z]);
 		put4(off_tail, labels_crc);
 		e.device_stream_bytes = 0;
-		if (e.keep_device_stream) {
+		if (sealed) e.device_stream_bytes = total;
+		else if (e.keep_device_stream) {
 			e.d_stream_out.ensure(total + 16);
 			uint8_t* ds = e.d_stream_out.p;
 			const void* up = head.label_format == FLAT ? o : nullptr;
@@ -2329,8 +2538,8 @@
 			else CKL_HIP(hipMemcpyAsync(o + off_codes, e.d_codes_out.p, cr.total, hipMemcpyDeviceToHost, s));
 		}
 		ht.mark("assembly");
-		CKL_HIP(hipEventRecord(e.ev1, s));
-		CKL_HIP(hipStreamSynchronize(s));
+		if (!sealed) CKL_HIP(hipEventRecord(e.ev1, s));
+		if (!sealed || (cr.total && !e.async_host_copy)) CKL_HIP(hipStreamSynchronize(s));
 		ht.mark("codes_d2h");
 		CKL_HIP(hipGetLastError());
 		CKL_HIP(hipEventElapsedTime(&e.pipeline_ms, e.ev0, e.ev1));
@@ -2690,6 +2899,26 @@
 	return CKL_OK;
 }
 
+int ckl_encoder_node_counts(ckl_encoder* e, uint32_t* counts, uint32_t max_slices, uint32_t* n_slices, int* from_planes, int* sized_from_planes) {
+	return guard([&] {
+		if (!e || !counts || !n_slices || !from_planes || !sized_from_planes) throw Error(CKL_ERR_ARG, "crackle_amd: null argument");
+		const size_t ns = e->last_trail_slices;
+		*n_slices = static_cast<uint32_t>(ns);
+		*from_planes = e->early_counts && e->early_special.size() == ns ? 1 : 0;
+		*sized_from_planes = e->early_counts_used ? 1 : 0;
+		if (!ns || !e->d_count_vh.p) { *n_slices = 0; return; }
+		if (ns > max_slices) throw Error(CKL_ERR_ARG, "crackle_amd: node counts need room for " + std::to_string(ns) + " slices");
+		select_device(e->device);
+		const std::vector<uint32_t> c = download(e->d_count_vh.p + 2 * ns, 2 * ns, e->stream);
+		for (size_t z = 0; z < ns; z++) {
+			counts[4 * z + 0] = *from_planes ? e->early_special[z] : 0u;
+			counts[4 * z + 1] = *from_planes ? e->early_corner[z] : 0u;
+			counts[4 * z + 2] = c[z];
+			counts[4 * z + 3] = c[ns + z];
+		}
+	});
+}
+
 int ckl_encoder_walk_step_kinds(ckl_encoder* e, uint32_t* counts, uint32_t max_slices, uint32_t* n_slices) {
 	return guard([&] {
 		if (!e || !counts || !n_slices) throw Error(CKL_ERR_ARG, "crackle_amd: null argument");
diff --git a/crackle_amd/csrc/ckl_encoder.hpp b/crackle_amd/csrc/ckl_encoder.hpp
--- a/crackle_amd/csrc/ckl_encoder.hpp
+++ b/crackle_amd/csrc/ckl_encoder.hpp
@@ -42,6 +42,11 @@
 	DevBuf<uint32_t> d_labels_crc;
 	DevBuf<uint8_t> d_stream_out;
 	uint64_t device_stream_bytes = 0;
+	DevBuf<uint32_t> d_seal_index;
+	DevBuf<uint32_t> d_seal_tail;
+	DevBuf<uint32_t> d_seal_crc;
+	void* report_staging = nullptr;
+	size_t report_staging_bytes = 0;
 	uint64_t last_codes_total = 0;
 	DevBuf<uint32_t> d_stack_node, d_stack_code;
 	DevBuf<uint32_t> d_chain_node, d_chain_off, d_chain_clen, d_chain_order, d_chain_dst, d_chain_vstart;
@@ -88,6 +93,11 @@
 	uint32_t tiles_x = 0, tiles_y = 0, mtx2 = 0;
 	uint64_t adjm_stride = 0;
 	bool graph_permissible = false;
+	DevBuf<uint32_t> d_plane_partial_nodes;
+	hipEvent_t ev_planes = nullptr;
+	bool early_counts = false;
+	bool early_counts_used = false;
+	std::vector<uint32_t> early_special, early_corner;
 	bool planes_deferred = false;
 	bool trail_zeroed = false;
 	DevBuf<uint64_t> t_nbase, t_cobase, t_ibase;
@@ -118,6 +128,8 @@
 		if (ev_codes) (void)hipEventDestroy(ev_codes);
 		if (tables_staging) ckl::host_out_free(tables_staging);
 		if (ev_labels_crc) (void)hipEventDestroy(ev_labels_crc);
+		if (ev_planes) (void)hipEventDestroy(ev_planes);
+		if (report_staging) ckl::host_out_free(report_staging);
 	}
 };
 
diff --git a/crackle_amd/csrc/ckl_trail.hpp b/crackle_amd/csrc/ckl_trail.hpp
--- a/crackle_amd/csrc/ckl_trail.hpp
+++ b/crackle_amd/csrc/ckl_trail.hpp
@@ -21,7 +21,7 @@
 	}
 };
 
-enum : uint32_t { TRAIL_ERR_CAPACITY = 1u };
+enum : uint32_t { TRAIL_ERR_CAPACITY = 1u, TRAIL_ERR_COUNTS = 2u  };
 constexpr uint32_t kDartNone = 0xFFFFFFFFu;
 constexpr uint32_t kItemSeg = 0u << 30, kItemCtl = 1u << 30, kItemDead = 2u << 30, kItemMask = 3u << 30;
 
@@ -242,7 +242,9 @@
 
 static __global__ void __launch_bounds__(kBlock) k_trail_count_scan(
 	uint32_t* __restrict__ blk_special, uint32_t* __restrict__ blk_corner, uint32_t nblk,
-	uint32_t* __restrict__ tot_special, uint32_t* __restrict__ tot_corner
+	uint32_t* __restrict__ tot_special, uint32_t* __restrict__ tot_corner,
+	const unsigned long long* __restrict__ expect, uint32_t perm_mode, const unsigned long long* __restrict__ total_pairs, unsigned long long half_voxels,
+	uint32_t* __restrict__ slice_err
 ) {
 	__shared__ uint32_t s_scan[2 * kWaves];
 	const uint32_t zi = blockIdx.x;
@@ -256,7 +258,13 @@
 		if (b < nblk) { bs[b] = cs + v[0]; bc[b] = cc + v[1]; }
 		cs += tot[0]; cc += tot[1];
 	}
-	if (threadIdx.x == 0) { tot_special[zi] = cs; tot_corner[zi] = cc; }
+	if (threadIdx.x == 0) {
+		tot_special[zi] = cs; tot_corner[zi] = cc;
+		if (expect) {
+			const bool permissible = perm_mode == 2u ? static_cast<long long>(*total_pairs) < static_cast<long long>(half_voxels) : perm_mode != 0u;
+			if (!permissible && (expect[2ull * zi] != cs || expect[2ull * zi + 1] != cc)) atomicOr(slice_err + zi, TRAIL_ERR_COUNTS);
+		}
+	}
 }
 
 static __global__ void __launch_bounds__(kBlock) k_trail_nodes(TrailArgs a) {
diff --git a/include/crackle_amd.h b/include/crackle_amd.h
--- a/include/crackle_amd.h
+++ b/include/crackle_amd.h
@@ -178,6 +178,7 @@
 int ckl_encoder_walk_paths(ckl_encoder* e, uint32_t* fast_slices, uint32_t* compiled_slices);
 int ckl_encoder_emit_path(const ckl_encoder* e, int* fused, uint64_t* lds_bytes);
 int ckl_encoder_walk_step_kinds(ckl_encoder* e, uint32_t* counts, uint32_t max_slices, uint32_t* n_slices);
+int ckl_encoder_node_counts(ckl_encoder* e, uint32_t* counts, uint32_t max_slices, uint32_t* n_slices, int* from_planes, int* sized_from_planes);
 void ckl_encoder_destroy(ckl_encoder* e);
 
 
```

Result: no change. 168.0 billion, median of 4 (+0.2%).
